# tczhangzhi/pytorch-distributed

Hardware: AMD Instinct MI355X
Metric: ImageNet images/sec (ResNet-50 train step, whole job) (higher is better)
Workload: dtype bf16; 1 GPU; model=resnet50, global_batch=3072, image_size=224, parallelism=dp1, style=ddp, hip_ext=True, hipgraph=False

## Files before the change

amdtrain/models/resnet.py:

```python

from __future__ import annotations

from typing import Callable, Dict, List, Optional, Type, Union

import torch
import torch.nn as nn

from ..ops import fused as OF


import os

from ..ops.conv import AmdConv2d, GradCell, ResidualGradTap
from ..ops.linear import AmdLinear


def _residual_fuse_enabled() -> bool:
    return os.environ.get("AMDTRAIN_RESFUSE", "1") == "1"


def conv3x3(in_planes: int, out_planes: int, stride: int = 1,
            groups: int = 1) -> nn.Conv2d:
    return AmdConv2d(in_planes, out_planes, kernel_size=3, stride=stride,
                     padding=1, groups=groups, bias=False)


def conv1x1(in_planes: int, out_planes: int, stride: int = 1) -> nn.Conv2d:
    return AmdConv2d(in_planes, out_planes, kernel_size=1, stride=stride,
                     bias=False)


class FusedBatchNorm2d(nn.BatchNorm2d):

    def forward(self, x: torch.Tensor) -> torch.Tensor:
        return OF.batch_norm(x, self, relu=False)

    def forward_relu(self, x: torch.Tensor) -> torch.Tensor:
        return OF.batch_norm(x, self, relu=True)


def _shortcut_tail(out: torch.Tensor, bn: FusedBatchNorm2d,
                   downsample: nn.Module, x: torch.Tensor) -> torch.Tensor:
    if (bn.training and isinstance(downsample, nn.Sequential)
            and len(downsample) == 2
            and isinstance(downsample[0], AmdConv2d)
            and isinstance(downsample[1], FusedBatchNorm2d)):
        return OF.bn_add_relu_downsample(out, bn, downsample[0](x),
                                         downsample[1])
    return OF.bn_add_relu(out, bn, downsample(x))


class BasicBlock(nn.Module):
    expansion = 1

    def __init__(self, inplanes: int, planes: int, stride: int = 1,
                 downsample: Optional[nn.Module] = None):
        super().__init__()
        self.conv1 = conv3x3(inplanes, planes, stride)
        self.bn1 = FusedBatchNorm2d(planes)
        self.relu = nn.ReLU(inplace=True)
        self.conv2 = conv3x3(planes, planes)
        self.bn2 = FusedBatchNorm2d(planes)
        self.downsample = downsample
        self.stride = stride

    def forward(self, x: torch.Tensor) -> torch.Tensor:
        identity = x
        cell = None
        if (self.training and x.is_cuda and torch.is_grad_enabled()
                and _residual_fuse_enabled()):
            cell = getattr(x, "_amdtrain_next_cell", None)
        out = self.bn1.forward_relu(self.conv1(x))
        out = self.conv2(out)
        if cell is not None:
            cell.armed = True
            identity = ResidualGradTap.apply(x, cell)
        if self.downsample is not None:
            return _shortcut_tail(out, self.bn2, self.downsample, identity)
        return OF.bn_add_relu(out, self.bn2, identity)


class Bottleneck(nn.Module):
    expansion = 4

    def __init__(self, inplanes: int, planes: int, stride: int = 1,
                 downsample: Optional[nn.Module] = None, groups: int = 1,
                 base_width: int = 64):
        super().__init__()
        width = int(planes * (base_width / 64.0)) * groups
        self.conv1 = conv1x1(inplanes, width)
        self.bn1 = FusedBatchNorm2d(width)
        self.conv2 = conv3x3(width, width, stride, groups)
        self.bn2 = FusedBatchNorm2d(width)
        self.conv3 = conv1x1(width, planes * self.expansion)
        self.bn3 = FusedBatchNorm2d(planes * self.expansion)
        self.relu = nn.ReLU(inplace=True)
        self.downsample = downsample
        self.stride = stride

    def forward(self, x: torch.Tensor) -> torch.Tensor:
        identity = x
        cell = None
        if (self.training and x.is_cuda and torch.is_grad_enabled()
                and _residual_fuse_enabled()):
            cell = getattr(x, "_amdtrain_next_cell", None)
        out = self.bn1.forward_relu(self.conv1(x))
        out = self.bn2.forward_relu(self.conv2(out))
        out = self.conv3(out)
        if cell is not None:
            cell.armed = True
            identity = ResidualGradTap.apply(x, cell)
        if self.downsample is not None:
            return _shortcut_tail(out, self.bn3, self.downsample, identity)
        return OF.bn_add_relu(out, self.bn3, identity)


class ResNet(nn.Module):
    def __init__(self, block: Type[Union[BasicBlock, Bottleneck]],
                 layers: List[int], num_classes: int = 1000,
                 zero_init_residual: bool = False, groups: int = 1,
                 width_per_group: int = 64):
        super().__init__()
        self.groups = groups
        self.base_width = width_per_group
        self.inplanes = 64
        self.conv1 = AmdConv2d(3, 64, kernel_size=7, stride=2, padding=3,
                               bias=False)
        self.bn1 = FusedBatchNorm2d(64)
        self.relu = nn.ReLU(inplace=True)
        self.maxpool = nn.MaxPool2d(kernel_size=3, stride=2, padding=1)
        self.layer1 = self._make_layer(block, 64, layers[0])
        self.layer2 = self._make_layer(block, 128, layers[1], stride=2)
        self.layer3 = self._make_layer(block, 256, layers[2], stride=2)
        self.layer4 = self._make_layer(block, 512, layers[3], stride=2)
        self.avgpool = nn.AdaptiveAvgPool2d((1, 1))
        self.fc = AmdLinear(512 * block.expansion, num_classes)

        for m in self.modules():
            if isinstance(m, nn.Conv2d):
                nn.init.kaiming_normal_(m.weight, mode="fan_out",
                                        nonlinearity="relu")
            elif isinstance(m, nn.BatchNorm2d):
                nn.init.constant_(m.weight, 1)
                nn.init.constant_(m.bias, 0)
        if zero_init_residual:
            for m in self.modules():
                if isinstance(m, Bottleneck):
                    nn.init.constant_(m.bn3.weight, 0)
                elif isinstance(m, BasicBlock):
                    nn.init.constant_(m.bn2.weight, 0)

    def _make_layer(self, block, planes: int, blocks: int,
                    stride: int = 1) -> nn.Sequential:
        downsample = None
        if stride != 1 or self.inplanes != planes * block.expansion:
            downsample = nn.Sequential(
                conv1x1(self.inplanes, planes * block.expansion, stride),
                FusedBatchNorm2d(planes * block.expansion),
            )
        kw = {}
        if block is Bottleneck:
            kw = dict(groups=self.groups, base_width=self.base_width)
        layers = [block(self.inplanes, planes, stride, downsample, **kw)]
        self.inplanes = planes * block.expansion
        for _ in range(1, blocks):
            layers.append(block(self.inplanes, planes, **kw))
        return nn.Sequential(*layers)

    def forward(self, x: torch.Tensor) -> torch.Tensor:
        x = OF.bn_relu_max_pool(self.conv1(x), self.bn1)
        x = self.layer1(x)
        x = self.layer2(x)
        x = self.layer3(x)
        x = self.layer4(x)
        x = OF.global_avg_pool(x)
        x = torch.flatten(x, 1)
        return self.fc(x)


def resnet18(num_classes: int = 1000, **kw) -> ResNet:
    return ResNet(BasicBlock, [2, 2, 2, 2], num_classes=num_classes, **kw)


def resnet34(num_classes: int = 1000, **kw) -> ResNet:
    return ResNet(BasicBlock, [3, 4, 6, 3], num_classes=num_classes, **kw)


def resnet50(num_classes: int = 1000, **kw) -> ResNet:
    return ResNet(Bottleneck, [3, 4, 6, 3], num_classes=num_classes, **kw)


def resnet101(num_classes: int = 1000, **kw) -> ResNet:
    return ResNet(Bottleneck, [3, 4, 23, 3], num_classes=num_classes, **kw)


def resnet152(num_classes: int = 1000, **kw) -> ResNet:
    return ResNet(Bottleneck, [3, 8, 36, 3], num_classes=num_classes, **kw)


def resnext50_32x4d(num_classes: int = 1000, **kw) -> ResNet:
    return ResNet(Bottleneck, [3, 4, 6, 3], num_classes=num_classes,
                  groups=32, width_per_group=4, **kw)


def wide_resnet50_2(num_classes: int = 1000, **kw) -> ResNet:
    return ResNet(Bottleneck, [3, 4, 6, 3], num_classes=num_classes,
                  width_per_group=128, **kw)


_REGISTRY: Dict[str, Callable[..., nn.Module]] = {
    "resnet18": resnet18,
    "resnet34": resnet34,
    "resnet50": resnet50,
    "resnet101": resnet101,
    "resnet152": resnet152,
    "resnext50_32x4d": resnext50_32x4d,
    "wide_resnet50_2": wide_resnet50_2,
}


def model_names() -> List[str]:
    return sorted(_REGISTRY)


def build_model(arch: str, num_classes: int = 1000, **kw) -> nn.Module:
    if arch not in _REGISTRY:
        raise ValueError(f"unknown arch '{arch}'; choices: {model_names()}")
    return _REGISTRY[arch](num_classes=num_classes, **kw)
```

amdtrain/ops/conv.py:

```python

from __future__ import annotations

import os

import torch
import torch.nn as nn

from ._ext import ext_available, require_ext


def _rows(x: torch.Tensor) -> torch.Tensor:
    n, c, h, w = x.shape
    return x.permute(0, 2, 3, 1).reshape(n * h * w, c)


def _fuse_stats_enabled() -> bool:
    return os.environ.get("AMDTRAIN_FUSE_BNSTATS", "1") == "1"


def _wgrad2_enabled() -> bool:
    return os.environ.get("AMDTRAIN_WGRAD2", "1") == "1"


class GradCell:
    __slots__ = ("armed", "g")

    def __init__(self):
        self.armed = False
        self.g = None


class ResidualGradTap(torch.autograd.Function):

    @staticmethod
    def forward(ctx, z: torch.Tensor, cell: "GradCell"):
        ctx.cell = cell
        return z.view_as(z)

    @staticmethod
    def backward(ctx, grad: torch.Tensor):
        if ctx.cell.armed:
            ctx.cell.g = grad
            return None, None
        return grad, None


class _Conv1x1(torch.autograd.Function):

    @staticmethod
    @torch.amp.custom_fwd(device_type="cuda", cast_inputs=torch.bfloat16)
    def forward(ctx, x: torch.Tensor, weight: torch.Tensor, stride: int):
        e = require_ext()
        n, cin, h, w = x.shape
        cout = weight.shape[0]
        xc = x.contiguous(memory_format=torch.channels_last)
        x2d = _rows(xc)
        w2d = weight.reshape(cout, cin)
        stats = None
        if stride > 1:
            y2d = e.gemm_bt_strided(x2d, w2d, n, h, w, stride)
            ho = (h + stride - 1) // stride
            wo = (w + stride - 1) // stride
        elif _fuse_stats_enabled():
            y2d, stats = e.gemm_bt_stats(x2d, w2d)
            ho, wo = h, w
        else:
            y2d = e.gemm_bt(x2d, w2d, False)
            ho, wo = h, w
        ctx.save_for_backward(x2d, w2d)
        ctx.meta = (n, cin, h, w, stride, ho, wo, cout)
        y = y2d.view(n, ho, wo, cout).permute(0, 3, 1, 2)
        if stats is None:
            stats = torch.empty(0, device=x.device)
        ctx.mark_non_differentiable(stats)
        return y, stats

    @staticmethod
    @torch.amp.custom_bwd(device_type="cuda")
    def backward(ctx, grad_y: torch.Tensor, _grad_stats=None):
        e = require_ext()
        x2d, w2d = ctx.saved_tensors
        n, cin, h, w, stride, ho, wo, cout = ctx.meta
        gy = grad_y.contiguous(memory_format=torch.channels_last)
        gy2d = _rows(gy).to(torch.bfloat16)
        wT = e.transpose_2d(w2d)
        dx2d = e.gemm_bt(gy2d, wT, False)
        if stride > 1:
            dx = e.scatter_rows_x2(dx2d, n, h, w, ho, wo)
            dw = e.tn2_wgrad(gy2d, x2d, 1, n, h, w, stride, 1) \
                if _wgrad2_enabled() \
                else e.gemm_tn_strided(gy2d, x2d, n, h, w, stride)
        else:
            dx = dx2d.view(n, ho, wo, cin).permute(0, 3, 1, 2)
            dw = e.tn2_wgrad(gy2d, x2d) if _wgrad2_enabled() \
                else e.gemm_tn(gy2d, x2d, 0)
        return dx, dw.reshape(cout, cin, 1, 1), None


def conv1x1_mfma(x: torch.Tensor, weight: torch.Tensor,
                 stride: int = 1) -> torch.Tensor:
    y, stats = _Conv1x1.apply(x, weight, stride)
    if stats.numel():
        y._amdtrain_bn_stats = stats
    return y


class _Conv3x3(torch.autograd.Function):

    @staticmethod
    @torch.amp.custom_fwd(device_type="cuda", cast_inputs=torch.bfloat16)
    def forward(ctx, x: torch.Tensor, weight: torch.Tensor, stride: int):
        e = require_ext()
        n, cin, h, w = x.shape
        cout = weight.shape[0]
        xc = x.contiguous(memory_format=torch.channels_last)
        x2d = _rows(xc)
        w2d = weight.contiguous(memory_format=torch.channels_last) \
            .permute(0, 2, 3, 1).reshape(cout, 9 * cin)
        if _fuse_stats_enabled():
            y2d, stats = e.conv3x3_fwd_stats(x2d, n, h, w, stride, w2d)
        else:
            y2d = e.conv3x3_fwd(x2d, n, h, w, stride, w2d)
            stats = torch.empty(0, device=x.device)
        ctx.save_for_backward(x2d, w2d)
        ctx.meta = (n, cin, h, w, stride, cout)
        ho = (h + 2 - 3) // stride + 1
        wo = (w + 2 - 3) // stride + 1
        y = y2d.view(n, ho, wo, cout).permute(0, 3, 1, 2)
        ctx.mark_non_differentiable(stats)
        return y, stats

    @staticmethod
    @torch.amp.custom_bwd(device_type="cuda")
    def backward(ctx, grad_y: torch.Tensor, _grad_stats=None):
        e = require_ext()
        x2d, w2d = ctx.saved_tensors
        n, cin, h, w, stride, cout = ctx.meta
        gy = grad_y.contiguous(memory_format=torch.channels_last)
        gy2d = _rows(gy).to(torch.bfloat16)
        dx2d = e.conv3x3_dgrad(gy2d, n, h, w, stride, w2d)
        dx = dx2d.view(n, h, w, cin).permute(0, 3, 1, 2)
        dw2d = e.tn2_wgrad(gy2d, x2d, 9, n, h, w, stride, 2) \
            if _wgrad2_enabled() \
            else e.conv3x3_wgrad(gy2d, x2d, n, h, w, stride)
        dw = dw2d.view(cout, 3, 3, cin).permute(0, 3, 1, 2) \
            .contiguous(memory_format=torch.channels_last)
        return dx, dw, None


def conv3x3_mfma(x: torch.Tensor, weight: torch.Tensor,
                 stride: int = 1) -> torch.Tensor:
    y, stats = _Conv3x3.apply(x, weight, stride)
    if stats.numel():
        y._amdtrain_bn_stats = stats
    return y


class _ConvGrouped3x3(torch.autograd.Function):

    @staticmethod
    @torch.amp.custom_fwd(device_type="cuda", cast_inputs=torch.bfloat16)
    def forward(ctx, x: torch.Tensor, weight: torch.Tensor, stride: int,
                groups: int):
        e = require_ext()
        n, cin, h, w = x.shape
        cout = weight.shape[0]
        sg = cin // groups
        xc = x.contiguous(memory_format=torch.channels_last)
        x2d = _rows(xc)
        sout = cout // groups
        wg = weight.contiguous(memory_format=torch.channels_last) \
            .permute(0, 2, 3, 1).reshape(groups, sout, 3, 3, sg)
        dense = torch.zeros(groups, sout, 3, 3, groups, sg,
                            dtype=wg.dtype, device=wg.device)
        gi = torch.arange(groups, device=wg.device)
        dense[gi, :, :, :, gi, :] = wg
        w2d = dense.reshape(cout, 3, 3, cin).reshape(cout, 9 * cin)
        banded = (cin == cout and cin % 128 == 0)
        if _fuse_stats_enabled():
            y2d, stats = e.conv3x3_fwd_stats(x2d, n, h, w, stride, w2d,
                                             banded)
        else:
            y2d = e.conv3x3_fwd(x2d, n, h, w, stride, w2d)
            stats = torch.empty(0, device=x.device)
        ctx.save_for_backward(x2d, w2d)
        ctx.meta = (n, cin, h, w, stride, cout, groups, banded)
        ho = (h + 2 - 3) // stride + 1
        wo = (w + 2 - 3) // stride + 1
        y = y2d.view(n, ho, wo, cout).permute(0, 3, 1, 2)
        ctx.mark_non_differentiable(stats)
        return y, stats

    @staticmethod
    @torch.amp.custom_bwd(device_type="cuda")
    def backward(ctx, grad_y: torch.Tensor, _grad_stats=None):
        e = require_ext()
        x2d, w2d = ctx.saved_tensors
        n, cin, h, w, stride, cout, groups, banded = ctx.meta
        sg = cin // groups
        sout = cout // groups
        gy = grad_y.contiguous(memory_format=torch.channels_last)
        gy2d = _rows(gy).to(torch.bfloat16)
        dx2d = e.conv3x3_dgrad(gy2d, n, h, w, stride, w2d, banded)
        dx = dx2d.view(n, h, w, cin).permute(0, 3, 1, 2)
        if banded and _wgrad2_enabled():
            dwb = e.tn2_wgrad_banded(gy2d, x2d, n, h, w, stride) \
                .view(cout // 128, 128 // sg, sg, 9, 128 // sg, sg)
            bi = torch.arange(cout // 128, device=dwb.device)[:, None]
            gi = torch.arange(128 // sg, device=dwb.device)[None, :]
            dw = dwb[bi, gi, :, :, gi, :].reshape(cout, 9, sg) \
                .view(cout, 3, 3, sg).permute(0, 3, 1, 2) \
                .contiguous(memory_format=torch.channels_last)
            return dx, dw, None, None
        dw2d = e.tn2_wgrad(gy2d, x2d, 9, n, h, w, stride, 2) \
            if _wgrad2_enabled() \
            else e.conv3x3_wgrad(gy2d, x2d, n, h, w, stride)
        dwd = dw2d.view(groups, sout, 3, 3, groups, sg)
        gi = torch.arange(groups, device=dwd.device)
        dw = dwd[gi, :, :, :, gi, :].permute(0, 1, 4, 2, 3) \
            .reshape(cout, sg, 3, 3) \
            .contiguous(memory_format=torch.channels_last)
        return dx, dw, None, None


def conv3x3_grouped_mfma(x: torch.Tensor, weight: torch.Tensor,
                         stride: int, groups: int) -> torch.Tensor:
    y, stats = _ConvGrouped3x3.apply(x, weight, stride, groups)
    if stats.numel():
        y._amdtrain_bn_stats = stats
    return y


class _ConvGeneric(torch.autograd.Function):

    @staticmethod
    @torch.amp.custom_fwd(device_type="cuda", cast_inputs=torch.bfloat16)
    def forward(ctx, x: torch.Tensor, weight: torch.Tensor, stride: int,
                pad: int):
        e = require_ext()
        n, cin, h, w = x.shape
        cout, _, kh, kw = weight.shape
        xc = x.contiguous(memory_format=torch.channels_last)
        x2d = _rows(xc)
        w4 = weight.contiguous(memory_format=torch.channels_last) \
            .permute(0, 2, 3, 1)
        if cin < 8:
            x2d = torch.nn.functional.pad(x2d, (0, 8 - cin))
            w4 = torch.nn.functional.pad(w4, (0, 8 - cin))
            cin_k = 8
        else:
            cin_k = cin
        k = kh * kw * cin_k
        kpad = (k + 31) // 32 * 32
        w2 = w4.reshape(cout, k)
        if kpad != k:
            w2 = torch.nn.functional.pad(w2, (0, kpad - k))
        y2d = e.conv_generic_fwd(x2d, n, h, w, kh, kw, stride, pad, w2)
        ctx.save_for_backward(x2d, weight)
        ctx.meta = (n, cin, h, w, kh, kw, stride, pad, cout, k, cin_k)
        ho = (h + 2 * pad - kh) // stride + 1
        wo = (w + 2 * pad - kw) // stride + 1
        return y2d.view(n, ho, wo, cout).permute(0, 3, 1, 2)

    @staticmethod
    @torch.amp.custom_bwd(device_type="cuda")
    def backward(ctx, grad_y: torch.Tensor):
        e = require_ext()
        x2d, weight = ctx.saved_tensors
        n, cin, h, w, kh, kw, stride, pad, cout, k, cin_k = ctx.meta
        gy2d = _rows(grad_y.contiguous(memory_format=torch.channels_last)) \
            .to(torch.bfloat16)
        dx = None
        if ctx.needs_input_grad[0]:
            k2 = kh * kw * cout
            k2p = (k2 + 31) // 32 * 32
            w2p = weight.to(torch.bfloat16).permute(1, 2, 3, 0) \
                .reshape(cin, k2)
            if k2p != k2:
                w2p = torch.nn.functional.pad(w2p, (0, k2p - k2))
            dx2d = e.conv_generic_dgrad(gy2d, w2p.contiguous(), n, h, w,
                                        kh, kw, stride, pad)
            dx = dx2d.view(n, h, w, cin).permute(0, 3, 1, 2)
        if _wgrad2_enabled() and cout % 8 == 0:
            dwp = e.tn2_wgrad(gy2d, x2d, kh * kw, n, h, w, stride, 2,
                              kh, kw, pad)
            dw = dwp.view(cout, kh * kw, cin_k)[:, :, :cin] \
                .view(cout, kh, kw, cin).permute(0, 3, 1, 2) \
                .contiguous(memory_format=torch.channels_last)
        else:
            dw2 = e.conv_generic_wgrad(gy2d, x2d, n, h, w, kh, kw, stride,
                                       pad)
            dw = dw2[:, :k].view(cout, kh * kw, cin_k)[:, :, :cin] \
                .reshape(cout, kh, kw, cin).permute(0, 3, 1, 2) \
                .contiguous(memory_format=torch.channels_last)
        return dx, dw, None, None


def conv_stem_mfma(x: torch.Tensor, weight: torch.Tensor, stride: int,
                   pad: int) -> torch.Tensor:
    return _ConvGeneric.apply(x, weight, stride, pad)


def _conv1x1_env_default() -> str:
    return os.environ.get("AMDTRAIN_CONV1X1", "custom")


class AmdConv2d(nn.Conv2d):

    def forward(self, x: torch.Tensor) -> torch.Tensor:
        bf16_ok = (x.dtype == torch.bfloat16
                   or torch.is_autocast_enabled("cuda"))
        if (x.is_cuda and bf16_ok and ext_available()
                and self.bias is None and self.dilation == (1, 1)
                and self.groups > 1):
            if (self.kernel_size == (3, 3) and self.padding == (1, 1)
                    and self.stride[0] in (1, 2)
                    and self.in_channels % 32 == 0
                    and self.out_channels % 16 == 0
                    and self.in_channels % self.groups == 0
                    and os.environ.get("AMDTRAIN_CONV3X3G", "custom")
                    == "custom"):
                return conv3x3_grouped_mfma(x, self.weight, self.stride[0],
                                            self.groups)
            return super().forward(x)
        if (x.is_cuda and bf16_ok and ext_available()
                and self.bias is None and self.groups == 1
                and self.dilation == (1, 1)):
            ch_ok = (self.in_channels % 32 == 0
                     and self.out_channels % 16 == 0)
            if (ch_ok and self.kernel_size == (1, 1)
                    and self.padding == (0, 0)
                    and _conv1x1_env_default() == "custom"):
                return conv1x1_mfma(x, self.weight, self.stride[0])
            if (ch_ok and self.kernel_size == (3, 3)
                    and self.padding == (1, 1)
                    and self.stride[0] in (1, 2)
                    and os.environ.get("AMDTRAIN_CONV3X3", "custom")
                    == "custom"):
                return conv3x3_mfma(x, self.weight, self.stride[0])
            if (self.out_channels % 16 == 0
                    and self.stride[0] == self.stride[1]
                    and self.padding[0] == self.padding[1]
                    and os.environ.get("AMDTRAIN_CONVSTEM", "custom")
                    == "custom"):
                return conv_stem_mfma(x, self.weight, self.stride[0],
                                      self.padding[0])
        return super().forward(x)
```

amdtrain/ops/csrc/batchnorm.hip:

```cpp
#include "common.h"

namespace {

template <typename T>
struct BNDualSide {
  const T* x = nullptr;
  const float* mean = nullptr;
  const float* invstd = nullptr;
  float* out = nullptr;
};

template <typename T, int VEC, bool BWD, int MASK, bool WG, bool GO2,
          bool DUAL = false>
__global__ void __launch_bounds__(AMD_TPB)
bn_reduce_kernel(const T* __restrict__ x, const T* __restrict__ go,
                 const T* __restrict__ goB, const T* __restrict__ y,
                 const float* __restrict__ mean,
                 const float* __restrict__ invstd,
                 const float* __restrict__ scale,
                 const float* __restrict__ shift, T* __restrict__ ghat_out,
                 float* __restrict__ out, long R, int C,
                 BNDualSide<T> ds = {}) {
  static_assert(!DUAL || (BWD && WG), "DUAL rides the ghat-writing bwd pass");
  const int t = threadIdx.x;
  const int gpr = C / VEC;
  const long rows_per_block = (R + gridDim.x - 1) / gridDim.x;
  const long r0 = blockIdx.x * rows_per_block;
  const long r1 = min(r0 + rows_per_block, R);

  if (gpr <= AMD_TPB) {
    const int gc = t % gpr;
    const int phase = t / gpr;
    const int rstep = AMD_TPB / gpr;
    const int c0 = gc * VEC;
    float sa[VEC], sb[VEC];
#pragma unroll
    for (int k = 0; k < VEC; ++k) sa[k] = sb[k] = 0.f;
    float mk[VEC], ik[VEC], sck[VEC], shk[VEC];
    float sda[VEC], sdb[VEC], mdk[VEC], idk[VEC];
    if (BWD) {
#pragma unroll
      for (int k = 0; k < VEC; ++k) {
        mk[k] = mean[c0 + k];
        ik[k] = invstd[c0 + k];
        if (MASK == 2) {
          sck[k] = scale[c0 + k];
          shk[k] = shift[c0 + k];
        }
        if (DUAL) {
          sda[k] = sdb[k] = 0.f;
          mdk[k] = ds.mean[c0 + k];
          idk[k] = ds.invstd[c0 + k];
        }
      }
    }
    for (long r = r0 + phase; r < r1; r += rstep) {
      const long base = r * C + c0;
      Pack<T, VEC> xv = *(const Pack<T, VEC>*)(x + base);
      Pack<T, VEC> gv, gv2, yv, gh, dv;
      unsigned int mbits = 0;
      if (BWD) {
        gv = *(const Pack<T, VEC>*)(go + base);
        if (DUAL) dv = *(const Pack<T, VEC>*)(ds.x + base);
        if (GO2) gv2 = *(const Pack<T, VEC>*)(goB + base);
        if (MASK == 1) yv = *(const Pack<T, VEC>*)(y + base);
        if (MASK == 3)
          mbits = ((const unsigned char*)y)[base / VEC];
      }
#pragma unroll
      for (int k = 0; k < VEC; ++k) {
        float xe = to_f32(xv.v[k]);
        if (BWD) {
          float ge = to_f32(gv.v[k]);
          if (GO2) ge += to_f32(gv2.v[k]);
          if (MASK == 1 && to_f32(yv.v[k]) <= 0.f) ge = 0.f;
          if (MASK == 2 && sck[k] * xe + shk[k] <= 0.f) ge = 0.f;
          if (MASK == 3 && !(mbits & (1u << k))) ge = 0.f;
          sa[k] += ge;
          sb[k] += ge * (xe - mk[k]) * ik[k];
          if (WG) gh.v[k] = from_f32<T>(ge);
          if (DUAL) {
            const float gr = to_f32(gh.v[k]);
            sda[k] += gr;
            sdb[k] += gr * (to_f32(dv.v[k]) - mdk[k]) * idk[k];
          }
        } else {
          sa[k] += xe;
          sb[k] += xe * xe;
        }
      }
      if (BWD && WG) *(Pack<T, VEC>*)(ghat_out + base) = gh;
    }
    __shared__ float lds[AMD_TPB * VEC];
    auto fold = [&](float(&s)[VEC]) {
#pragma unroll
      for (int k = 0; k < VEC; ++k) lds[t * VEC + k] = s[k];
      __syncthreads();
      if (phase == 0) {
        for (int ph = 1; ph < rstep; ++ph)
#pragma unroll
          for (int k = 0; k < VEC; ++k)
            s[k] += lds[(ph * gpr + gc) * VEC + k];
      }
      __syncthreads();
    };
    fold(sa);
    fold(sb);
    if (DUAL) {
      fold(sda);
      fold(sdb);
    }
    if (phase == 0) {
      float* part = out + (long)blockIdx.x * 2 * C;
#pragma unroll
      for (int k = 0; k < VEC; ++k) {
        part[c0 + k] = sa[k];
        part[C + c0 + k] = sb[k];
      }
      if (DUAL) {
        float* partd = ds.out + (long)blockIdx.x * 2 * C;
#pragma unroll
        for (int k = 0; k < VEC; ++k) {
          partd[c0 + k] = sda[k];
          partd[C + c0 + k] = sdb[k];
        }
      }
    }
  } else {
    const int cpt = gpr / AMD_TPB;
    float sa[2][VEC], sb[2][VEC];
    float mk[2][VEC], ik[2][VEC], sck[2][VEC], shk[2][VEC];
#pragma unroll
    for (int j = 0; j < 2; ++j)
#pragma unroll
      for (int k = 0; k < VEC; ++k) {
        sa[j][k] = sb[j][k] = 0.f;
        if (BWD && j < cpt) {
          mk[j][k] = mean[(t + j * AMD_TPB) * VEC + k];
          ik[j][k] = invstd[(t + j * AMD_TPB) * VEC + k];
          if (MASK == 2) {
            sck[j][k] = scale[(t + j * AMD_TPB) * VEC + k];
            shk[j][k] = shift[(t + j * AMD_TPB) * VEC + k];
          }
        }
      }
    for (long r = r0; r < r1; ++r) {
      for (int j = 0; j < cpt; ++j) {
        const int c0 = (t + j * AMD_TPB) * VEC;
        const long base = r * C + c0;
        Pack<T, VEC> xv = *(const Pack<T, VEC>*)(x + base);
        Pack<T, VEC> gv, gv2, yv, gh;
        unsigned int mbits = 0;
        if (BWD) {
          gv = *(const Pack<T, VEC>*)(go + base);
          if (GO2) gv2 = *(const Pack<T, VEC>*)(goB + base);
          if (MASK == 1) yv = *(const Pack<T, VEC>*)(y + base);
          if (MASK == 3)
            mbits = ((const unsigned char*)y)[base / VEC];
        }
#pragma unroll
        for (int k = 0; k < VEC; ++k) {
          float xe = to_f32(xv.v[k]);
          if (BWD) {
            float ge = to_f32(gv.v[k]);
            if (GO2) ge += to_f32(gv2.v[k]);
            if (MASK == 1 && to_f32(yv.v[k]) <= 0.f) ge = 0.f;
            if (MASK == 2 && sck[j][k] * xe + shk[j][k] <= 0.f) ge = 0.f;
            if (MASK == 3 && !(mbits & (1u << k))) ge = 0.f;
            sa[j][k] += ge;
            sb[j][k] += ge * (xe - mk[j][k]) * ik[j][k];
            if (WG) gh.v[k] = from_f32<T>(ge);
          } else {
            sa[j][k] += xe;
            sb[j][k] += xe * xe;
          }
        }
        if (BWD && WG) *(Pack<T, VEC>*)(ghat_out + base) = gh;
      }
    }
    float* part = out + (long)blockIdx.x * 2 * C;
    for (int j = 0; j < cpt; ++j) {
      const int c0 = (t + j * AMD_TPB) * VEC;
#pragma unroll
      for (int k = 0; k < VEC; ++k) {
        part[c0 + k] = sa[j][k];
        part[C + c0 + k] = sb[j][k];
      }
    }
  }
}

constexpr int BN_COLLAPSE = 32;

static inline int bn_collapse_slots(int nparts) {
  return nparts >= 2048 ? 4 * BN_COLLAPSE : BN_COLLAPSE;
}

__global__ void bn_collapse_partials_kernel(const float* __restrict__ in,
                                            float* __restrict__ out,
                                            int nparts, int twoC, int slots) {
  const int slot = blockIdx.x % slots;
  const int cblk = blockIdx.x / slots;
  const int c = cblk * AMD_TPB + threadIdx.x;
  if (c >= twoC) return;
  float acc = 0.f;
  for (int p = slot; p < nparts; p += slots)
    acc += in[(long)p * twoC + c];
  out[(long)slot * twoC + c] = acc;
}

__global__ void bn_finalize_train_kernel(
    const float* __restrict__ partials, int nparts,
    const float* __restrict__ w,
    const float* __restrict__ b, float* __restrict__ rm,
    float* __restrict__ rv, float* __restrict__ mean,
    float* __restrict__ invstd, float* __restrict__ scale,
    float* __restrict__ shift, long R, int C, float momentum, float eps) {
  const int c = blockIdx.x * 64 + (threadIdx.x & 63);
  const int sl = threadIdx.x >> 6;
  float s1 = 0.f, s2 = 0.f;
  if (c < C)
    for (int p = sl; p < nparts; p += 4) {
      s1 += partials[(long)p * 2 * C + c];
      s2 += partials[(long)p * 2 * C + C + c];
    }
  __shared__ float red[2][4][64];
  red[0][sl][threadIdx.x & 63] = s1;
  red[1][sl][threadIdx.x & 63] = s2;
  __syncthreads();
  if (sl != 0 || c >= C) return;
  s1 += red[0][1][threadIdx.x] + red[0][2][threadIdx.x] +
        red[0][3][threadIdx.x];
  s2 += red[1][1][threadIdx.x] + red[1][2][threadIdx.x] +
        red[1][3][threadIdx.x];
  float m = s1 / R;
  float var = fmaxf(s2 / R - m * m, 0.f);
  float is = rsqrtf(var + eps);
  mean[c] = m;
  invstd[c] = is;
  float unbiased = R > 1 ? var * (float)R / (float)(R - 1) : var;
  rm[c] = (1.f - momentum) * rm[c] + momentum * m;
  rv[c] = (1.f - momentum) * rv[c] + momentum * unbiased;
  float sc = w[c] * is;
  scale[c] = sc;
  shift[c] = b[c] - m * sc;
}

__global__ void bn_finalize_eval_kernel(
    const float* __restrict__ w, const float* __restrict__ b,
    const float* __restrict__ rm, const float* __restrict__ rv,
    float* __restrict__ scale, float* __restrict__ shift, int C, float eps) {
  int c = blockIdx.x * blockDim.x + threadIdx.x;
  if (c >= C) return;
  float is = rsqrtf(rv[c] + eps);
  float sc = w[c] * is;
  scale[c] = sc;
  shift[c] = b[c] - rm[c] * sc;
}

template <typename T, int VEC, bool RELU, bool HAS_ADD, bool POW2,
          bool DUAL = false>
__global__ void __launch_bounds__(AMD_TPB)
bn_apply_kernel(const T* __restrict__ x, const T* __restrict__ z,
                T* __restrict__ y, unsigned char* __restrict__ mask,
                const float* __restrict__ scale,
                const float* __restrict__ shift, long total_vec, int C,
                const float* __restrict__ scale_d = nullptr,
                const float* __restrict__ shift_d = nullptr) {
  static_assert(!DUAL || (HAS_ADD && POW2), "DUAL normalizes the addend");
  extern __shared__ float sm[];
  const int gpr = C / VEC;
  const long stride = (long)gridDim.x * blockDim.x;
  float rs[VEC], rb[VEC], rsd[VEC], rbd[VEC];
  if (DUAL) {
    const int cf =
        (int)(((long)blockIdx.x * blockDim.x + threadIdx.x) & (gpr - 1)) * VEC;
#pragma unroll
    for (int k = 0; k < VEC; ++k) {
      rs[k] = scale[cf + k];
      rb[k] = shift[cf + k];
      rsd[k] = scale_d[cf + k];
      rbd[k] = shift_d[cf + k];
    }
  } else {
    for (int c = threadIdx.x; c < C; c += blockDim.x) {
      sm[c] = scale[c];
      sm[C + c] = shift[c];
    }
    __syncthreads();
  }
  for (long i = (long)blockIdx.x * blockDim.x + threadIdx.x; i < total_vec;
       i += 2 * stride) {
    const bool has2 = i + stride < total_vec;
    const long i2 = has2 ? i + stride : i;
    Pack<T, VEC> xv = *(const Pack<T, VEC>*)(x + i * VEC);
    Pack<T, VEC> xv2 = *(const Pack<T, VEC>*)(x + i2 * VEC);
    Pack<T, VEC> zv, zv2;
    if (HAS_ADD) {
      zv = *(const Pack<T, VEC>*)(z + i * VEC);
      zv2 = *(const Pack<T, VEC>*)(z + i2 * VEC);
    }
    const int c0 = (int)(POW2 ? (i & (gpr - 1)) : (i % gpr)) * VEC;
    const int c02 = (int)(POW2 ? (i2 & (gpr - 1)) : (i2 % gpr)) * VEC;
    Pack<T, VEC> yv, yv2;
    unsigned int mb = 0, mb2 = 0;
#pragma unroll
    for (int k = 0; k < VEC; ++k) {
      float v = DUAL ? rs[k] * to_f32(xv.v[k]) + rb[k]
                     : sm[c0 + k] * to_f32(xv.v[k]) + sm[C + c0 + k];
      if (HAS_ADD) {
        float ze = to_f32(zv.v[k]);
        if (DUAL) ze = to_f32(from_f32<T>(rsd[k] * ze + rbd[k]));
        v += ze;
      }
      if (RELU) {
        if (mask != nullptr && v > 0.f) mb |= 1u << k;
        v = fmaxf(v, 0.f);
      }
      yv.v[k] = from_f32<T>(v);
      float v2 = DUAL ? rs[k] * to_f32(xv2.v[k]) + rb[k]
                      : sm[c02 + k] * to_f32(xv2.v[k]) + sm[C + c02 + k];
      if (HAS_ADD) {
        float ze2 = to_f32(zv2.v[k]);
        if (DUAL) ze2 = to_f32(from_f32<T>(rsd[k] * ze2 + rbd[k]));
        v2 += ze2;
      }
      if (RELU) {
        if (mask != nullptr && v2 > 0.f) mb2 |= 1u << k;
        v2 = fmaxf(v2, 0.f);
      }
      yv2.v[k] = from_f32<T>(v2);
    }
    *(Pack<T, VEC>*)(y + i * VEC) = yv;
    if (has2) *(Pack<T, VEC>*)(y + i2 * VEC) = yv2;
    if (RELU && mask != nullptr) {
      mask[i] = (unsigned char)mb;
      if (has2) mask[i2] = (unsigned char)mb2;
    }
  }
}

__global__ void bn_bwd_finalize_kernel(
    const float* __restrict__ partials, int nparts,
    const float* __restrict__ w, const float* __restrict__ mean,
    const float* __restrict__ invstd, float* __restrict__ gw,
    float* __restrict__ gb, float* __restrict__ A, float* __restrict__ Bc,
    float* __restrict__ Dc, long R, int C) {
  const int c = blockIdx.x * 64 + (threadIdx.x & 63);
  const int sl = threadIdx.x >> 6;
  float sg = 0.f, sgx = 0.f;
  if (c < C)
    for (int p = sl; p < nparts; p += 4) {
      sg += partials[(long)p * 2 * C + c];
      sgx += partials[(long)p * 2 * C + C + c];
    }
  __shared__ float red[2][4][64];
  red[0][sl][threadIdx.x & 63] = sg;
  red[1][sl][threadIdx.x & 63] = sgx;
  __syncthreads();
  if (sl != 0 || c >= C) return;
  sg += red[0][1][threadIdx.x] + red[0][2][threadIdx.x] +
        red[0][3][threadIdx.x];
  sgx += red[1][1][threadIdx.x] + red[1][2][threadIdx.x] +
         red[1][3][threadIdx.x];
  gb[c] = sg;
  gw[c] = sgx;
  float a = w[c] * invstd[c];
  float bcoef = -a * invstd[c] * sgx / R;
  A[c] = a;
  Bc[c] = bcoef;
  Dc[c] = -a * sg / R - bcoef * mean[c];
}

template <typename T>
struct BNDualBwdSide {
  const T* x = nullptr;
  T* gx = nullptr;
  const float* A = nullptr;
  const float* Bc = nullptr;
  const float* Dc = nullptr;
};

template <typename T, int VEC, int MASK, bool WRITE_GHAT, bool POW2,
          bool DUAL = false>
__global__ void __launch_bounds__(AMD_TPB)
bn_bwd_apply_kernel(const T* __restrict__ x, const T* __restrict__ go,
                    T* __restrict__ gx,
                    T* __restrict__ ghat_out, const float* __restrict__ A,
                    const float* __restrict__ Bc, const float* __restrict__ Dc,
                    const float* __restrict__ scale,
                    const float* __restrict__ shift, long total_vec, int C,
                    BNDualBwdSide<T> ds = {}) {
  static_assert(!DUAL || (MASK == 0 && POW2 && !WRITE_GHAT),
                "DUAL consumes the materialized ghat");
  const int gpr = C / VEC;
  const long stride = (long)gridDim.x * blockDim.x;
  if (DUAL) {
    const long i0 = (long)blockIdx.x * blockDim.x + threadIdx.x;
    const int c0 = (int)(i0 & (gpr - 1)) * VEC;
    float a3[VEC], b3[VEC], d3[VEC], ad[VEC], bd[VEC], dd[VEC];
#pragma unroll
    for (int k = 0; k < VEC; ++k) {
      a3[k] = A[c0 + k];
      b3[k] = Bc[c0 + k];
      d3[k] = Dc[c0 + k];
      ad[k] = ds.A[c0 + k];
      bd[k] = ds.Bc[c0 + k];
      dd[k] = ds.Dc[c0 + k];
    }
    for (long i = i0; i < total_vec; i += 2 * stride) {
      const bool has2 = i + stride < total_vec;
      const long i2 = has2 ? i + stride : i;
      Pack<T, VEC> xv = *(const Pack<T, VEC>*)(x + i * VEC);
      Pack<T, VEC> dv = *(const Pack<T, VEC>*)(ds.x + i * VEC);
      Pack<T, VEC> gv = *(const Pack<T, VEC>*)(go + i * VEC);
      Pack<T, VEC> xv2 = *(const Pack<T, VEC>*)(x + i2 * VEC);
      Pack<T, VEC> dv2 = *(const Pack<T, VEC>*)(ds.x + i2 * VEC);
      Pack<T, VEC> gv2 = *(const Pack<T, VEC>*)(go + i2 * VEC);
      Pack<T, VEC> out, dout, out2, dout2;
#pragma unroll
      for (int k = 0; k < VEC; ++k) {
        float ge = to_f32(gv.v[k]);
        float v = a3[k] * ge + b3[k] * to_f32(xv.v[k]) + d3[k];
        out.v[k] = from_f32<T>(v);
        float w = ad[k] * ge + bd[k] * to_f32(dv.v[k]) + dd[k];
        dout.v[k] = from_f32<T>(w);
        float ge2 = to_f32(gv2.v[k]);
        float v2 = a3[k] * ge2 + b3[k] * to_f32(xv2.v[k]) + d3[k];
        out2.v[k] = from_f32<T>(v2);
        float w2 = ad[k] * ge2 + bd[k] * to_f32(dv2.v[k]) + dd[k];
        dout2.v[k] = from_f32<T>(w2);
      }
      *(Pack<T, VEC>*)(gx + i * VEC) = out;
      *(Pack<T, VEC>*)(ds.gx + i * VEC) = dout;
      if (has2) {
        *(Pack<T, VEC>*)(gx + i2 * VEC) = out2;
        *(Pack<T, VEC>*)(ds.gx + i2 * VEC) = dout2;
      }
    }
    return;
  }
  extern __shared__ float sm[];
  for (int c = threadIdx.x; c < C; c += blockDim.x) {
    sm[c] = A[c];
    sm[C + c] = Bc[c];
    sm[2 * C + c] = Dc[c];
    if (MASK == 2) {
      sm[3 * C + c] = scale[c];
      sm[4 * C + c] = shift[c];
    }
  }
  __syncthreads();
  for (long i = (long)blockIdx.x * blockDim.x + threadIdx.x; i < total_vec;
       i += 2 * stride) {
    const bool has2 = i + stride < total_vec;
    const long i2 = has2 ? i + stride : i;
    Pack<T, VEC> xv = *(const Pack<T, VEC>*)(x + i * VEC);
    Pack<T, VEC> gv = *(const Pack<T, VEC>*)(go + i * VEC);
    Pack<T, VEC> xv2 = *(const Pack<T, VEC>*)(x + i2 * VEC);
    Pack<T, VEC> gv2 = *(const Pack<T, VEC>*)(go + i2 * VEC);
    const int c0 = (int)(POW2 ? (i & (gpr - 1)) : (i % gpr)) * VEC;
    const int c02 = (int)(POW2 ? (i2 & (gpr - 1)) : (i2 % gpr)) * VEC;
    Pack<T, VEC> out, gh, out2, gh2;
#pragma unroll
    for (int k = 0; k < VEC; ++k) {
      float xe = to_f32(xv.v[k]);
      float ge = to_f32(gv.v[k]);
      if (MASK == 2 && sm[3 * C + c0 + k] * xe + sm[4 * C + c0 + k] <= 0.f)
        ge = 0.f;
      float v = sm[c0 + k] * ge + sm[C + c0 + k] * xe + sm[2 * C + c0 + k];
      out.v[k] = from_f32<T>(v);
      if (WRITE_GHAT) gh.v[k] = from_f32<T>(ge);
      float xe2 = to_f32(xv2.v[k]);
      float ge2 = to_f32(gv2.v[k]);
      if (MASK == 2 && sm[3 * C + c02 + k] * xe2 + sm[4 * C + c02 + k] <= 0.f)
        ge2 = 0.f;
      float v2 = sm[c02 + k] * ge2 + sm[C + c02 + k] * xe2 +
                 sm[2 * C + c02 + k];
      out2.v[k] = from_f32<T>(v2);
      if (WRITE_GHAT) gh2.v[k] = from_f32<T>(ge2);
    }
    *(Pack<T, VEC>*)(gx + i * VEC) = out;
    if (WRITE_GHAT) *(Pack<T, VEC>*)(ghat_out + i * VEC) = gh;
    if (has2) {
      *(Pack<T, VEC>*)(gx + i2 * VEC) = out2;
      if (WRITE_GHAT) *(Pack<T, VEC>*)(ghat_out + i2 * VEC) = gh2;
    }
  }
}


static void check_nhwc(const at::Tensor& x) {
  TORCH_CHECK(x.is_cuda() && x.dim() == 4, "expected 4D CUDA tensor");
  TORCH_CHECK(x.is_contiguous(at::MemoryFormat::ChannelsLast),
              "expected channels_last (NHWC) tensor");
}

template <typename F>
static void dispatch_vec(const at::Tensor& x, F fn) {
  int C = (int)x.size(1);
  AT_DISPATCH_FLOATING_TYPES_AND2(
      at::ScalarType::BFloat16, at::ScalarType::Half, x.scalar_type(), "bn",
      [&] {
        using devT = typename DevT<scalar_t>::type;
        constexpr int VEC = 16 / sizeof(devT);
        TORCH_CHECK(C % VEC == 0, "C must be a multiple of ", VEC);
        TORCH_CHECK((C & (C - 1)) == 0,
                    "C must be a power of two (apply-kernel fast path): ", C);
        TORCH_CHECK(C / VEC <= 2 * AMD_TPB, "C too large: ", C);
        fn((devT*)nullptr, std::integral_constant<int, VEC>{});
      });
}

static int bn_reduce_grid(long R, int C) {
  long rows_per_block = std::max<long>(1, R / 1536);
  return (int)std::min<long>((R + rows_per_block - 1) / rows_per_block, 1536);
}

static at::Tensor bn_collapse(const at::Tensor& parts, long C,
                              hipStream_t stream) {
  const int nparts = (int)parts.size(0);
  const int slots = bn_collapse_slots(nparts);
  auto sums2 = at::empty({slots, 2 * C}, parts.options());
  int cgrid = slots * (int)((2 * C + AMD_TPB - 1) / AMD_TPB);
  bn_collapse_partials_kernel<<<cgrid, AMD_TPB, 0, stream>>>(
      parts.data_ptr<float>(), sums2.data_ptr<float>(), nparts, (int)(2 * C),
      slots);
  CHECK_CUDA_OK();
  return sums2;
}

struct BNTrainStats {
  at::Tensor mean, invstd, scale, shift;
};

static BNTrainStats bn_train_stats(const at::Tensor& x,
                                   const std::optional<at::Tensor>& parts,
                                   const at::Tensor& weight,
                                   const at::Tensor& bias,
                                   at::Tensor& running_mean,
                                   at::Tensor& running_var, double momentum,
                                   double eps) {
  const long C = x.size(1);
  const long R = x.numel() / C;
  auto opts = x.options().dtype(at::kFloat);
  auto stream = at::cuda::getCurrentCUDAStream();
  at::Tensor sums;
  if (parts) {
    TORCH_CHECK(parts->size(1) == 2 * C, "parts must be [nparts][2C]");
    sums = *parts;
  } else {
    const int rgrid = bn_reduce_grid(R, C);
    sums = at::empty({rgrid, 2 * C}, opts);
    dispatch_vec(x, [&](auto* tp, auto vec) {
      using devT = std::remove_pointer_t<decltype(tp)>;
      constexpr int VEC = decltype(vec)::value;
      bn_reduce_kernel<devT, VEC, false, 0, false, false>
          <<<rgrid, AMD_TPB, 0, stream>>>((const devT*)x.const_data_ptr(),
                                          nullptr, nullptr, nullptr, nullptr,
                                          nullptr, nullptr, nullptr, nullptr,
                                          sums.data_ptr<float>(), R, (int)C);
      CHECK_CUDA_OK();
    });
  }
  auto sums2 = bn_collapse(sums, C, stream);
  BNTrainStats s{at::empty({C}, opts), at::empty({C}, opts),
                 at::empty({C}, opts), at::empty({C}, opts)};
  int fgrid = (int)((C + 63) / 64);
  bn_finalize_train_kernel<<<fgrid, AMD_TPB, 0, stream>>>(
      sums2.data_ptr<float>(), (int)sums2.size(0), weight.data_ptr<float>(),
      bias.data_ptr<float>(), running_mean.data_ptr<float>(),
      running_var.data_ptr<float>(), s.mean.data_ptr<float>(),
      s.invstd.data_ptr<float>(), s.scale.data_ptr<float>(),
      s.shift.data_ptr<float>(), R, (int)C, (float)momentum, (float)eps);
  CHECK_CUDA_OK();
  return s;
}

struct BNBwdCoeffs {
  at::Tensor gw, gb, A, Bc, Dc;
};

static BNBwdCoeffs bn_bwd_coeffs(const at::Tensor& sums,
                                 const at::Tensor& weight,
                                 const at::Tensor& mean,
                                 const at::Tensor& invstd, long R, long C) {
  auto stream = at::cuda::getCurrentCUDAStream();
  auto opts = sums.options();
  auto sums2 = bn_collapse(sums, C, stream);
  BNBwdCoeffs k{at::empty({C}, opts), at::empty({C}, opts),
                at::empty({C}, opts), at::empty({C}, opts),
                at::empty({C}, opts)};
  int fgrid = (int)((C + 63) / 64);
  bn_bwd_finalize_kernel<<<fgrid, AMD_TPB, 0, stream>>>(
      sums2.data_ptr<float>(), (int)sums2.size(0), weight.data_ptr<float>(),
      mean.data_ptr<float>(), invstd.data_ptr<float>(),
      k.gw.data_ptr<float>(), k.gb.data_ptr<float>(), k.A.data_ptr<float>(),
      k.Bc.data_ptr<float>(), k.Dc.data_ptr<float>(), R, (int)C);
  CHECK_CUDA_OK();
  return k;
}

static void check_dual(const at::Tensor& x3, const at::Tensor& x_d) {
  check_nhwc(x3);
  check_nhwc(x_d);
  TORCH_CHECK(x3.sizes() == x_d.sizes() &&
                  x3.scalar_type() == x_d.scalar_type(),
              "dual BN tail: x3 and x_d must match in shape and dtype");
  TORCH_CHECK(x3.size(1) * (long)x3.element_size() / 16 <= AMD_TPB,
              "dual BN tail: C too wide for the register path: ", x3.size(1));
}

}

std::vector<at::Tensor> batch_norm_train_stats(
    at::Tensor x, std::optional<at::Tensor> parts, at::Tensor weight,
    at::Tensor bias, at::Tensor running_mean, at::Tensor running_var,
    double momentum, double eps) {
  check_nhwc(x);
  auto s = bn_train_stats(x, parts, weight, bias, running_mean, running_var,
                          momentum, eps);
  return {s.mean, s.invstd, s.scale, s.shift};
}

std::vector<at::Tensor> batch_norm_fwd_train(
    at::Tensor x, at::Tensor weight, at::Tensor bias, at::Tensor running_mean,
    at::Tensor running_var, double momentum, double eps, bool relu,
    std::optional<at::Tensor> addend) {
  check_nhwc(x);
  const long N = x.size(0), C = x.size(1), H = x.size(2), W = x.size(3);
  const long R = N * H * W;
  auto y = at::empty_like(x);
  at::Tensor mask;
  if (relu && addend)
    mask = at::empty({R * C / 4}, x.options().dtype(at::kByte));
  auto stream = at::cuda::getCurrentCUDAStream();
  auto st = bn_train_stats(x, std::nullopt, weight, bias, running_mean,
                           running_var, momentum, eps);
  auto &mean = st.mean, &invstd = st.invstd, &scale = st.scale,
       &shift = st.shift;

  dispatch_vec(x, [&](auto* tp, auto vec) {
    using devT = std::remove_pointer_t<decltype(tp)>;
    constexpr int VEC = decltype(vec)::value;
    long total_vec = R * C / VEC;
    int agrid = amd_grid(total_vec);
    size_t smem = 2 * C * sizeof(float);
    const devT* zp =
        addend ? (const devT*)addend->const_data_ptr() : nullptr;
#define APPLY(RELU_, ADD_)                                                  \
  bn_apply_kernel<devT, VEC, RELU_, ADD_, true>                             \
      <<<agrid, AMD_TPB, smem, stream>>>(                                   \
          (const devT*)x.const_data_ptr(), zp, (devT*)y.data_ptr(),         \
          mask.defined() ? mask.data_ptr<unsigned char>() : nullptr,        \
          scale.data_ptr<float>(), shift.data_ptr<float>(),     \
          total_vec, (int)C)
    if (relu && addend) APPLY(true, true);
    else if (relu) APPLY(true, false);
    else if (addend) APPLY(false, true);
    else APPLY(false, false);
#undef APPLY
    CHECK_CUDA_OK();
  });
  if (!mask.defined()) mask = at::empty({0}, x.options().dtype(at::kByte));
  return {y, mean, invstd, scale, shift, mask};
}

std::vector<at::Tensor> batch_norm_fwd_train_from_parts(
    at::Tensor x, at::Tensor parts, at::Tensor weight, at::Tensor bias,
    at::Tensor running_mean, at::Tensor running_var, double momentum,
    double eps, bool relu, std::optional<at::Tensor> addend) {
  check_nhwc(x);
  const long C = x.size(1);
  const long R = x.numel() / C;
  auto y = at::empty_like(x);
  at::Tensor mask;
  if (relu && addend)
    mask = at::empty({R * C / 4}, x.options().dtype(at::kByte));
  auto stream = at::cuda::getCurrentCUDAStream();
  auto st = bn_train_stats(x, parts, weight, bias, running_mean, running_var,
                           momentum, eps);
  auto &mean = st.mean, &invstd = st.invstd, &scale = st.scale,
       &shift = st.shift;
  dispatch_vec(x, [&](auto* tp, auto vec) {
    using devT = std::remove_pointer_t<decltype(tp)>;
    constexpr int VEC = decltype(vec)::value;
    long total_vec = R * C / VEC;
    int agrid = amd_grid(total_vec);
    size_t smem = 2 * C * sizeof(float);
    const devT* zp =
        addend ? (const devT*)addend->const_data_ptr() : nullptr;
#define APPLY2(RELU_, ADD_)                                                 \
  bn_apply_kernel<devT, VEC, RELU_, ADD_, true>                             \
      <<<agrid, AMD_TPB, smem, stream>>>(                                   \
          (const devT*)x.const_data_ptr(), zp, (devT*)y.data_ptr(),         \
          mask.defined() ? mask.data_ptr<unsigned char>() : nullptr,        \
          scale.data_ptr<float>(), shift.data_ptr<float>(),                 \
          total_vec, (int)C)
    if (relu && addend) APPLY2(true, true);
    else if (relu) APPLY2(true, false);
    else if (addend) APPLY2(false, true);
    else APPLY2(false, false);
#undef APPLY2
    CHECK_CUDA_OK();
  });
  if (!mask.defined()) mask = at::empty({0}, x.options().dtype(at::kByte));
  return {y, mean, invstd, scale, shift, mask};
}

std::vector<at::Tensor> batch_norm_dual_fwd_train(
    at::Tensor x3, at::Tensor x_d, std::optional<at::Tensor> parts3,
    std::optional<at::Tensor> parts_d, at::Tensor weight3, at::Tensor bias3,
    at::Tensor running_mean3, at::Tensor running_var3, double momentum3,
    double eps3, at::Tensor weight_d, at::Tensor bias_d,
    at::Tensor running_mean_d, at::Tensor running_var_d, double momentum_d,
    double eps_d) {
  check_dual(x3, x_d);
  const long C = x3.size(1);
  const long R = x3.numel() / C;
  auto sd = bn_train_stats(x_d, parts_d, weight_d, bias_d, running_mean_d,
                           running_var_d, momentum_d, eps_d);
  auto s3 = bn_train_stats(x3, parts3, weight3, bias3, running_mean3,
                           running_var3, momentum3, eps3);
  auto y = at::empty_like(x3);
  auto mask = at::empty({R * C / 4}, x3.options().dtype(at::kByte));
  auto stream = at::cuda::getCurrentCUDAStream();
  dispatch_vec(x3, [&](auto* tp, auto vec) {
    using devT = std::remove_pointer_t<decltype(tp)>;
    constexpr int VEC = decltype(vec)::value;
    long total_vec = R * C / VEC;
    int agrid = amd_grid(total_vec);
    bn_apply_kernel<devT, VEC, true, true, true, true>
        <<<agrid, AMD_TPB, 0, stream>>>(
            (const devT*)x3.const_data_ptr(),
            (const devT*)x_d.const_data_ptr(), (devT*)y.data_ptr(),
            mask.data_ptr<unsigned char>(), s3.scale.data_ptr<float>(),
            s3.shift.data_ptr<float>(), total_vec, (int)C,
            sd.scale.data_ptr<float>(), sd.shift.data_ptr<float>());
    CHECK_CUDA_OK();
  });
  return {y, s3.mean, s3.invstd, sd.mean, sd.invstd, mask};
}

std::vector<at::Tensor> batch_norm_dual_bwd(
    at::Tensor x3, at::Tensor x_d, at::Tensor grad_out,
    std::optional<at::Tensor> grad_out2, at::Tensor relu_mask,
    at::Tensor weight3, at::Tensor mean3, at::Tensor invstd3,
    at::Tensor weight_d, at::Tensor mean_d, at::Tensor invstd_d) {
  check_dual(x3, x_d);
  check_nhwc(grad_out);
  const long C = x3.size(1);
  const long R = x3.numel() / C;
  TORCH_CHECK(relu_mask.numel() == R * C / 4, "relu_mask size mismatch");
  auto opts = x3.options().dtype(at::kFloat);
  const int rgrid = bn_reduce_grid(R, C);
  auto sums3 = at::empty({rgrid, 2 * C}, opts);
  auto sums_d = at::empty({rgrid, 2 * C}, opts);
  auto ghat = at::empty_like(grad_out);
  auto gx3 = at::empty_like(x3);
  auto gx_d = at::empty_like(x_d);
  BNBwdCoeffs k3, kd;
  auto stream = at::cuda::getCurrentCUDAStream();
  dispatch_vec(x3, [&](auto* tp, auto vec) {
    using devT = std::remove_pointer_t<decltype(tp)>;
    constexpr int VEC = decltype(vec)::value;
    const devT* go2p = grad_out2
        ? (const devT*)grad_out2->const_data_ptr() : nullptr;
    BNDualSide<devT> rs{(const devT*)x_d.const_data_ptr(),
                        mean_d.data_ptr<float>(), invstd_d.data_ptr<float>(),
                        sums_d.data_ptr<float>()};
#define REDUCE_DUAL(GO2_)                                                   \
  bn_reduce_kernel<devT, VEC, true, 3, true, GO2_, true>                    \
      <<<rgrid, AMD_TPB, 0, stream>>>(                                      \
          (const devT*)x3.const_data_ptr(),                                 \
          (const devT*)grad_out.const_data_ptr(), go2p,                     \
          (const devT*)relu_mask.const_data_ptr(), mean3.data_ptr<float>(), \
          invstd3.data_ptr<float>(), nullptr, nullptr,                      \
          (devT*)ghat.data_ptr(), sums3.data_ptr<float>(), R, (int)C, rs)
    if (go2p) REDUCE_DUAL(true);
    else REDUCE_DUAL(false);
#undef REDUCE_DUAL
    CHECK_CUDA_OK();
    k3 = bn_bwd_coeffs(sums3, weight3, mean3, invstd3, R, C);
    kd = bn_bwd_coeffs(sums_d, weight_d, mean_d, invstd_d, R, C);
    long total_vec = R * C / VEC;
    int agrid = amd_grid(total_vec);
    BNDualBwdSide<devT> as{(const devT*)x_d.const_data_ptr(),
                           (devT*)gx_d.data_ptr(), kd.A.data_ptr<float>(),
                           kd.Bc.data_ptr<float>(), kd.Dc.data_ptr<float>()};
    bn_bwd_apply_kernel<devT, VEC, 0, false, true, true>
        <<<agrid, AMD_TPB, 0, stream>>>(
            (const devT*)x3.const_data_ptr(),
            (const devT*)ghat.const_data_ptr(), (devT*)gx3.data_ptr(),
            nullptr, k3.A.data_ptr<float>(), k3.Bc.data_ptr<float>(),
            k3.Dc.data_ptr<float>(), nullptr, nullptr, total_vec, (int)C, as);
    CHECK_CUDA_OK();
  });
  return {gx3, k3.gw, k3.gb, gx_d, kd.gw, kd.gb};
}

at::Tensor batch_norm_fwd_eval(at::Tensor x, at::Tensor weight,
                               at::Tensor bias, at::Tensor running_mean,
                               at::Tensor running_var, double eps, bool relu,
                               std::optional<at::Tensor> addend) {
  check_nhwc(x);
  const long C = x.size(1);
  const long R = x.numel() / C;
  auto opts = x.options().dtype(at::kFloat);
  auto scale = at::empty({C}, opts);
  auto shift = at::empty({C}, opts);
  auto y = at::empty_like(x);
  at::Tensor mask;
  auto stream = at::cuda::getCurrentCUDAStream();
  int fgrid = (int)((C + AMD_TPB - 1) / AMD_TPB);
  bn_finalize_eval_kernel<<<fgrid, AMD_TPB, 0, stream>>>(
      weight.data_ptr<float>(), bias.data_ptr<float>(),
      running_mean.data_ptr<float>(), running_var.data_ptr<float>(),
      scale.data_ptr<float>(), shift.data_ptr<float>(), (int)C, (float)eps);
  CHECK_CUDA_OK();
  dispatch_vec(x, [&](auto* tp, auto vec) {
    using devT = std::remove_pointer_t<decltype(tp)>;
    constexpr int VEC = decltype(vec)::value;
    long total_vec = R * C / VEC;
    int agrid = amd_grid(total_vec);
    size_t smem = 2 * C * sizeof(float);
    const devT* zp =
        addend ? (const devT*)addend->const_data_ptr() : nullptr;
#define APPLY(RELU_, ADD_)                                                  \
  bn_apply_kernel<devT, VEC, RELU_, ADD_, true>                             \
      <<<agrid, AMD_TPB, smem, stream>>>(                                   \
          (const devT*)x.const_data_ptr(), zp, (devT*)y.data_ptr(),         \
          mask.defined() ? mask.data_ptr<unsigned char>() : nullptr,        \
          scale.data_ptr<float>(), shift.data_ptr<float>(),     \
          total_vec, (int)C)
    if (relu && addend) APPLY(true, true);
    else if (relu) APPLY(true, false);
    else if (addend) APPLY(false, true);
    else APPLY(false, false);
#undef APPLY
    CHECK_CUDA_OK();
  });
  return y;
}

std::vector<at::Tensor> batch_norm_bwd(at::Tensor x, at::Tensor grad_out,
                                       std::optional<at::Tensor> y,
                                       at::Tensor weight,
                                       at::Tensor mean, at::Tensor invstd,
                                       bool relu, bool need_ghat,
                                       std::optional<at::Tensor> scale,
                                       std::optional<at::Tensor> shift,
                                       std::optional<at::Tensor> grad_out2,
                                       std::optional<at::Tensor> relu_mask) {
  check_nhwc(x);
  check_nhwc(grad_out);
  const long C = x.size(1);
  const long R = x.numel() / C;
  auto opts = x.options().dtype(at::kFloat);
  const int rgrid = bn_reduce_grid(R, C);
  auto sums = at::empty({rgrid, 2 * C}, opts);
  BNBwdCoeffs k;
  auto gx = at::empty_like(x);
  const bool affine_mask = relu && !need_ghat && scale && shift;
  const bool mask_y = relu && (!affine_mask || grad_out2.has_value());
  at::Tensor ghat;
  if (mask_y || grad_out2) ghat = at::empty_like(grad_out);
  auto stream = at::cuda::getCurrentCUDAStream();

  dispatch_vec(x, [&](auto* tp, auto vec) {
    using devT = std::remove_pointer_t<decltype(tp)>;
    constexpr int VEC = decltype(vec)::value;
    const float* scp = affine_mask ? scale->data_ptr<float>() : nullptr;
    const float* shp = affine_mask ? shift->data_ptr<float>() : nullptr;
    const devT* go2p = grad_out2
        ? (const devT*)grad_out2->const_data_ptr() : nullptr;
#define REDUCE(MASK_, WG_, GO2_)                                            \
  bn_reduce_kernel<devT, VEC, true, MASK_, WG_, GO2_>                       \
      <<<rgrid, AMD_TPB, 0, stream>>>(                                      \
          (const devT*)x.const_data_ptr(),                                  \
          (const devT*)grad_out.const_data_ptr(), go2p,                     \
          yp, mean.data_ptr<float>(),                                       \
          invstd.data_ptr<float>(), scp, shp,                               \
          WG_ ? (devT*)ghat.data_ptr() : nullptr,                           \
          sums.data_ptr<float>(), R, (int)C)
#define REDUCE3(GO2_)                                                       \
  bn_reduce_kernel<devT, VEC, true, 3, true, GO2_>                          \
      <<<rgrid, AMD_TPB, 0, stream>>>(                                      \
          (const devT*)x.const_data_ptr(),                                  \
          (const devT*)grad_out.const_data_ptr(), go2p,                     \
          (const devT*)mkp, mean.data_ptr<float>(),                         \
          invstd.data_ptr<float>(), scp, shp,                               \
          (devT*)ghat.data_ptr(),                                           \
          sums.data_ptr<float>(), R, (int)C)
    const unsigned char* mkp = (relu_mask && relu_mask->numel())
        ? relu_mask->data_ptr<unsigned char>() : nullptr;
    TORCH_CHECK(y.has_value() || !mask_y || mkp,
                "batch_norm_bwd: y is required to mask a relu+addend BN "
                "that saved no relu_mask");
    const devT* yp = y ? (const devT*)y->const_data_ptr() : nullptr;
    if (mask_y && mkp && go2p) REDUCE3(true);
    else if (mask_y && mkp) REDUCE3(false);
    else if (mask_y && go2p) REDUCE(1, true, true);
    else if (mask_y) REDUCE(1, true, false);
    else if (affine_mask) REDUCE(2, false, false);
    else if (go2p) REDUCE(0, true, true);
    else REDUCE(0, false, false);
#undef REDUCE
#undef REDUCE3
    CHECK_CUDA_OK();
    k = bn_bwd_coeffs(sums, weight, mean, invstd, R, C);
    long total_vec = R * C / VEC;
    int agrid = amd_grid(total_vec);
    size_t smem = (affine_mask ? 5 : 3) * C * sizeof(float);
    const devT* go_in = ghat.defined()
                            ? (const devT*)ghat.const_data_ptr()
                            : (const devT*)grad_out.const_data_ptr();
#define BAPPLY(MASK_)                                                       \
  bn_bwd_apply_kernel<devT, VEC, MASK_, false, true>                        \
      <<<agrid, AMD_TPB, smem, stream>>>(                                   \
          (const devT*)x.const_data_ptr(), go_in, (devT*)gx.data_ptr(),     \
          nullptr, k.A.data_ptr<float>(), k.Bc.data_ptr<float>(),           \
          k.Dc.data_ptr<float>(), scp, shp, total_vec, (int)C)
    if (affine_mask) BAPPLY(2);
    else BAPPLY(0);
#undef BAPPLY
    CHECK_CUDA_OK();
  });
  if (!ghat.defined()) ghat = grad_out;
  return {gx, k.gw, k.gb, ghat};
}
```

amdtrain/ops/csrc/ext.cpp:

```cpp
#include <torch/extension.h>

#include <optional>
#include <vector>

void multi_tensor_sgd(std::vector<at::Tensor> params,
                      std::vector<at::Tensor> grads,
                      std::vector<at::Tensor> momenta, double lr,
                      double momentum, double weight_decay, bool nesterov,
                      bool first, bool zero_grad);

std::vector<at::Tensor> cross_entropy_fwd(at::Tensor logits, at::Tensor target);
at::Tensor cross_entropy_bwd(at::Tensor logits, at::Tensor target,
                             at::Tensor lse, at::Tensor upstream);

at::Tensor normalize_u8(at::Tensor x, std::vector<double> mean,
                        std::vector<double> std_, long dtype_code);
at::Tensor topk_ranks(at::Tensor logits, at::Tensor target);
at::Tensor scatter_rows_x2(at::Tensor src2d, long Nn, long H, long W,
                           long Hs, long Ws);
void multi_tensor_scale_check(std::vector<at::Tensor> tensors, double scale,
                              at::Tensor found_inf);
void multi_tensor_cast(std::vector<at::Tensor> src,
                       std::vector<at::Tensor> dst);

std::vector<at::Tensor> batch_norm_fwd_train(
    at::Tensor x, at::Tensor weight, at::Tensor bias, at::Tensor running_mean,
    at::Tensor running_var, double momentum, double eps, bool relu,
    std::optional<at::Tensor> addend);
std::vector<at::Tensor> batch_norm_fwd_train_from_parts(
    at::Tensor x, at::Tensor parts, at::Tensor weight, at::Tensor bias,
    at::Tensor running_mean, at::Tensor running_var, double momentum,
    double eps, bool relu, std::optional<at::Tensor> addend);
at::Tensor batch_norm_fwd_eval(at::Tensor x, at::Tensor weight,
                               at::Tensor bias, at::Tensor running_mean,
                               at::Tensor running_var, double eps, bool relu,
                               std::optional<at::Tensor> addend);
std::vector<at::Tensor> batch_norm_train_stats(
    at::Tensor x, std::optional<at::Tensor> parts, at::Tensor weight,
    at::Tensor bias, at::Tensor running_mean, at::Tensor running_var,
    double momentum, double eps);
std::vector<at::Tensor> batch_norm_dual_fwd_train(
    at::Tensor x3, at::Tensor x_d, std::optional<at::Tensor> parts3,
    std::optional<at::Tensor> parts_d, at::Tensor weight3, at::Tensor bias3,
    at::Tensor running_mean3, at::Tensor running_var3, double momentum3,
    double eps3, at::Tensor weight_d, at::Tensor bias_d,
    at::Tensor running_mean_d, at::Tensor running_var_d, double momentum_d,
    double eps_d);
std::vector<at::Tensor> batch_norm_dual_bwd(
    at::Tensor x3, at::Tensor x_d, at::Tensor grad_out,
    std::optional<at::Tensor> grad_out2, at::Tensor relu_mask,
    at::Tensor weight3, at::Tensor mean3, at::Tensor invstd3,
    at::Tensor weight_d, at::Tensor mean_d, at::Tensor invstd_d);
std::vector<at::Tensor> batch_norm_bwd(at::Tensor x, at::Tensor grad_out,
                                       std::optional<at::Tensor> y,
                                       at::Tensor weight,
                                       at::Tensor mean, at::Tensor invstd,
                                       bool relu, bool need_ghat,
                                       std::optional<at::Tensor> scale,
                                       std::optional<at::Tensor> shift,
                                       std::optional<at::Tensor> grad_out2,
                                       std::optional<at::Tensor> relu_mask);

at::Tensor gemm_bt(at::Tensor A, at::Tensor B, bool f32_out,
                   std::optional<at::Tensor> addend,
                   std::optional<at::Tensor> bias);
at::Tensor gemm_tn(at::Tensor dY, at::Tensor X, long msplit);
at::Tensor gemm_bt_strided(at::Tensor A, at::Tensor B, long Nn, long H,
                           long W, long stride);
at::Tensor gemm_tn_strided(at::Tensor dY, at::Tensor X, long Nn, long H,
                           long W, long stride);
at::Tensor transpose_2d(at::Tensor x);

at::Tensor conv3x3_fwd(at::Tensor x2d, long Nn, long H, long W, long stride,
                       at::Tensor w2d);
std::vector<at::Tensor> conv3x3_fwd_stats(at::Tensor x2d, long Nn, long H,
                                          long W, long stride,
                                          at::Tensor w2d, bool banded);
std::vector<at::Tensor> gemm_bt_stats(at::Tensor A, at::Tensor B);

at::Tensor gemm_bt_8p(at::Tensor A, at::Tensor B);
at::Tensor gemm_bt_8p3(at::Tensor A, at::Tensor B);
at::Tensor conv3x3_8p(at::Tensor A2d, long Nn, long H, long W, long stride,
                      at::Tensor w2d, bool dgrad);
at::Tensor conv3x3_dgrad(at::Tensor dy2d, long Nn, long H, long W,
                         long stride, at::Tensor w2d, bool banded);
at::Tensor conv3x3_wgrad(at::Tensor dy2d, at::Tensor x2d, long Nn, long H,
                         long W, long stride);

at::Tensor tn2_wgrad(at::Tensor dY, at::Tensor X, long taps, long Nn, long H,
                     long W, long stride, long gmode, long kh, long kw,
                     long pad);
at::Tensor tn2_wgrad_banded(at::Tensor dY, at::Tensor X, long Nn, long H,
                            long W, long stride);
at::Tensor tr16_probe(at::Tensor in);

at::Tensor conv_generic_fwd(at::Tensor x2d, long Nn, long H, long W, long KH,
                            long KW, long stride, long pad, at::Tensor w2);
at::Tensor conv_generic_wgrad(at::Tensor dy2d, at::Tensor x2d, long Nn,
                              long H, long W, long KH, long KW, long stride,
                              long pad);
at::Tensor conv_generic_dgrad(at::Tensor dy2d, at::Tensor w2p, long Nn,
                              long H, long W, long KH, long KW, long stride,
                              long pad);

std::vector<at::Tensor> max_pool_3x3_s2_fwd(at::Tensor x,
                                            std::optional<at::Tensor> scale,
                                            std::optional<at::Tensor> shift);
at::Tensor max_pool_3x3_s2_bwd(at::Tensor grad_y, at::Tensor idx, long H,
                               long W);
at::Tensor global_avg_pool_fwd(at::Tensor x);
at::Tensor global_avg_pool_bwd(at::Tensor grad_y, long H, long W);

PYBIND11_MODULE(TORCH_EXTENSION_NAME, m) {
  m.doc() = "amdtrain hand-written gfx950 (CDNA4) HIP kernels";
  m.def("multi_tensor_sgd", &multi_tensor_sgd, "fused multi-tensor SGD");
  m.def("cross_entropy_fwd", &cross_entropy_fwd);
  m.def("cross_entropy_bwd", &cross_entropy_bwd);
  m.def("normalize_u8", &normalize_u8);
  m.def("topk_ranks", &topk_ranks);
  m.def("scatter_rows_x2", &scatter_rows_x2);
  m.def("multi_tensor_scale_check", &multi_tensor_scale_check);
  m.def("multi_tensor_cast", &multi_tensor_cast);
  m.def("batch_norm_fwd_train", &batch_norm_fwd_train,
        py::arg("x"), py::arg("weight"), py::arg("bias"),
        py::arg("running_mean"), py::arg("running_var"), py::arg("momentum"),
        py::arg("eps"), py::arg("relu"),
        py::arg("addend") = std::nullopt);
  m.def("batch_norm_fwd_train_from_parts", &batch_norm_fwd_train_from_parts,
        py::arg("x"), py::arg("parts"), py::arg("weight"), py::arg("bias"),
        py::arg("running_mean"), py::arg("running_var"), py::arg("momentum"),
        py::arg("eps"), py::arg("relu"), py::arg("addend") = std::nullopt);
  m.def("batch_norm_fwd_eval", &batch_norm_fwd_eval,
        py::arg("x"), py::arg("weight"), py::arg("bias"),
        py::arg("running_mean"), py::arg("running_var"), py::arg("eps"),
        py::arg("relu"), py::arg("addend") = std::nullopt);
  m.def("batch_norm_train_stats", &batch_norm_train_stats);
  m.def("batch_norm_dual_fwd_train", &batch_norm_dual_fwd_train);
  m.def("batch_norm_dual_bwd", &batch_norm_dual_bwd);
  m.def("batch_norm_bwd", &batch_norm_bwd, py::arg("x"), py::arg("grad_out"),
        py::arg("y"), py::arg("weight"), py::arg("mean"), py::arg("invstd"),
        py::arg("relu"), py::arg("need_ghat"),
        py::arg("scale") = std::nullopt, py::arg("shift") = std::nullopt,
        py::arg("grad_out2") = std::nullopt,
        py::arg("relu_mask") = std::nullopt);
  m.def("gemm_bt", &gemm_bt, py::arg("A"), py::arg("B"),
        py::arg("f32_out") = false, py::arg("addend") = std::nullopt,
        py::arg("bias") = std::nullopt);
  m.def("gemm_tn", &gemm_tn, py::arg("dY"), py::arg("X"),
        py::arg("msplit") = 0);
  m.def("gemm_bt_strided", &gemm_bt_strided);
  m.def("gemm_tn_strided", &gemm_tn_strided);
  m.def("transpose_2d", &transpose_2d);
  m.def("conv3x3_fwd", &conv3x3_fwd);
  m.def("conv3x3_fwd_stats", &conv3x3_fwd_stats, py::arg("x2d"),
        py::arg("Nn"), py::arg("H"), py::arg("W"), py::arg("stride"),
        py::arg("w2d"), py::arg("banded") = false);
  m.def("gemm_bt_stats", &gemm_bt_stats);
  m.def("gemm_bt_8p", &gemm_bt_8p);
  m.def("gemm_bt_8p3", &gemm_bt_8p3);
  m.def("conv3x3_8p", &conv3x3_8p);
  m.def("conv3x3_dgrad", &conv3x3_dgrad, py::arg("dy2d"), py::arg("Nn"),
        py::arg("H"), py::arg("W"), py::arg("stride"), py::arg("w2d"),
        py::arg("banded") = false);
  m.def("conv3x3_wgrad", &conv3x3_wgrad);
  m.def("tn2_wgrad", &tn2_wgrad, py::arg("dY"), py::arg("X"),
        py::arg("taps") = 1, py::arg("Nn") = 0, py::arg("H") = 0,
        py::arg("W") = 0, py::arg("stride") = 1, py::arg("gmode") = 0,
        py::arg("kh") = 3, py::arg("kw") = 3, py::arg("pad") = 1);
  m.def("tn2_wgrad_banded", &tn2_wgrad_banded);
  m.def("tr16_probe", &tr16_probe);
  m.def("conv_generic_fwd", &conv_generic_fwd);
  m.def("conv_generic_wgrad", &conv_generic_wgrad);
  m.def("conv_generic_dgrad", &conv_generic_dgrad);
  m.def("max_pool_3x3_s2_fwd", &max_pool_3x3_s2_fwd, py::arg("x"),
        py::arg("scale") = std::nullopt, py::arg("shift") = std::nullopt);
  m.def("max_pool_3x3_s2_bwd", &max_pool_3x3_s2_bwd);
  m.def("global_avg_pool_fwd", &global_avg_pool_fwd);
  m.def("global_avg_pool_bwd", &global_avg_pool_bwd);
}
```

amdtrain/ops/fused.py:

```python

from __future__ import annotations

import os
from typing import Optional

import torch
import torch.nn.functional as F

from ._ext import require_ext, use_ext_for
from .conv import GradCell

__all__ = ["batch_norm", "bn_add_relu", "bn_add_relu_downsample",
           "bn_relu_max_pool", "max_pool_3x3_s2", "global_avg_pool"]


class _BNFunction(torch.autograd.Function):

    @staticmethod
    def forward(ctx, x, weight, bias, running_mean, running_var,
                momentum, eps, relu, addend, parts, res_cell=None):
        e = require_ext()
        if parts is not None:
            y, mean, invstd, scale, shift, mask = \
                e.batch_norm_fwd_train_from_parts(
                    x, parts, weight, bias, running_mean, running_var,
                    float(momentum), float(eps), bool(relu), addend)
        else:
            y, mean, invstd, scale, shift, mask = e.batch_norm_fwd_train(
                x, weight, bias, running_mean, running_var,
                float(momentum), float(eps), bool(relu), addend)
        ctx.save_for_backward(x, y, weight, mean, invstd, scale, shift,
                              mask)
        ctx.relu = bool(relu)
        ctx.has_addend = addend is not None
        ctx.res_cell = res_cell
        return y

    @staticmethod
    def backward(ctx, grad_out):
        x, y, weight, mean, invstd, scale, shift, mask = ctx.saved_tensors
        e = require_ext()
        go2 = None
        cell = getattr(ctx, "res_cell", None)
        if cell is not None and cell.g is not None:
            go2 = cell.g.contiguous(memory_format=torch.channels_last)
            cell.g = None
        grad_x, grad_w, grad_b, ghat = e.batch_norm_bwd(
            x, grad_out.contiguous(memory_format=torch.channels_last),
            y, weight, mean, invstd, ctx.relu, ctx.has_addend,
            scale, shift, go2, mask)
        grad_addend = ghat if ctx.has_addend else None
        return (grad_x, grad_w, grad_b, None, None, None, None, None,
                grad_addend, None, None)


def _bn_torch(x: torch.Tensor, bn, relu: bool,
              addend: Optional[torch.Tensor]) -> torch.Tensor:
    y = F.batch_norm(
        x, bn.running_mean, bn.running_var, bn.weight, bn.bias,
        bn.training or not bn.track_running_stats,
        bn.momentum if bn.momentum is not None else 0.0, bn.eps)
    if addend is not None:
        y = y + addend
    if relu:
        y = F.relu(y, inplace=True)
    return y


def batch_norm(x: torch.Tensor, bn, relu: bool = False,
               addend: Optional[torch.Tensor] = None) -> torch.Tensor:
    if bn.training and bn.track_running_stats and bn.num_batches_tracked is not None:
        bn.num_batches_tracked.add_(1)
    C = x.size(1)
    if use_ext_for(x) and (C & (C - 1)) == 0:
        parts = getattr(x, "_amdtrain_bn_stats", None) if bn.training else None
        xc = x.contiguous(memory_format=torch.channels_last)
        ac = None if addend is None else addend.contiguous(memory_format=torch.channels_last)
        if bn.training:
            cell = GradCell() if (relu and ac is not None) else None
            out = _BNFunction.apply(xc, bn.weight, bn.bias, bn.running_mean,
                                    bn.running_var, bn.momentum, bn.eps,
                                    relu, ac, parts, cell)
            if cell is not None:
                out._amdtrain_next_cell = cell
            return out
        return require_ext().batch_norm_fwd_eval(
            xc, bn.weight, bn.bias, bn.running_mean, bn.running_var,
            float(bn.eps), bool(relu), ac)
    return _bn_torch(x, bn, relu, addend)


def bn_add_relu(x: torch.Tensor, bn, addend: torch.Tensor) -> torch.Tensor:
    return batch_norm(x, bn, relu=True, addend=addend)


class _BNDualFunction(torch.autograd.Function):

    @staticmethod
    def forward(ctx, x3, x_d, weight3, bias3, running_mean3, running_var3,
                momentum3, eps3, weight_d, bias_d, running_mean_d,
                running_var_d, momentum_d, eps_d, parts3, parts_d, res_cell):
        e = require_ext()
        y, mean3, invstd3, mean_d, invstd_d, mask = \
            e.batch_norm_dual_fwd_train(
                x3, x_d, parts3, parts_d,
                weight3, bias3, running_mean3, running_var3,
                float(momentum3), float(eps3),
                weight_d, bias_d, running_mean_d, running_var_d,
                float(momentum_d), float(eps_d))
        ctx.save_for_backward(x3, x_d, weight3, mean3, invstd3, weight_d,
                              mean_d, invstd_d, mask)
        ctx.res_cell = res_cell
        return y

    @staticmethod
    def backward(ctx, grad_out):
        (x3, x_d, weight3, mean3, invstd3, weight_d, mean_d, invstd_d,
         mask) = ctx.saved_tensors
        e = require_ext()
        go2 = None
        cell = getattr(ctx, "res_cell", None)
        if cell is not None and cell.g is not None:
            go2 = cell.g.contiguous(memory_format=torch.channels_last)
            cell.g = None
        gx3, gw3, gb3, gx_d, gw_d, gb_d = e.batch_norm_dual_bwd(
            x3, x_d, grad_out.contiguous(memory_format=torch.channels_last),
            go2, mask, weight3, mean3, invstd3, weight_d, mean_d, invstd_d)
        return (gx3, gx_d, gw3, gb3, None, None, None, None, gw_d, gb_d,
                None, None, None, None, None, None, None)


def _dsfuse_enabled() -> bool:
    return os.environ.get("AMDTRAIN_DSFUSE", "1") == "1"


def _stemfuse_enabled() -> bool:
    return os.environ.get("AMDTRAIN_STEMFUSE", "1") == "1"


def _vec_ok(x: torch.Tensor, max_groups: int) -> bool:
    C = x.size(1)
    vec = 16 // x.element_size()
    return (C & (C - 1)) == 0 and C % vec == 0 and C // vec <= max_groups


def bn_add_relu_downsample(x3: torch.Tensor, bn3, x_d: torch.Tensor,
                           bn_d) -> torch.Tensor:
    if (bn3.training and bn_d.training and _dsfuse_enabled()
            and use_ext_for(x3) and x3.shape == x_d.shape
            and x3.dtype == x_d.dtype and _vec_ok(x3, 256)):
        for bn in (bn_d, bn3):
            if bn.track_running_stats and bn.num_batches_tracked is not None:
                bn.num_batches_tracked.add_(1)
        parts3 = getattr(x3, "_amdtrain_bn_stats", None)
        parts_d = getattr(x_d, "_amdtrain_bn_stats", None)
        cell = GradCell()
        out = _BNDualFunction.apply(
            x3.contiguous(memory_format=torch.channels_last),
            x_d.contiguous(memory_format=torch.channels_last),
            bn3.weight, bn3.bias, bn3.running_mean, bn3.running_var,
            bn3.momentum, bn3.eps, bn_d.weight, bn_d.bias,
            bn_d.running_mean, bn_d.running_var, bn_d.momentum, bn_d.eps,
            parts3, parts_d, cell)
        out._amdtrain_next_cell = cell
        return out
    return bn_add_relu(x3, bn3, batch_norm(x_d, bn_d))


class _MaxPool3x3S2(torch.autograd.Function):
    @staticmethod
    def forward(ctx, x):
        e = require_ext()
        y, idx = e.max_pool_3x3_s2_fwd(x)
        ctx.save_for_backward(idx)
        ctx.in_shape = x.shape
        return y

    @staticmethod
    def backward(ctx, grad_out):
        (idx,) = ctx.saved_tensors
        e = require_ext()
        n, c, h, w = ctx.in_shape
        gx = e.max_pool_3x3_s2_bwd(
            grad_out.contiguous(memory_format=torch.channels_last), idx,
            int(h), int(w))
        return gx


def max_pool_3x3_s2(x: torch.Tensor) -> torch.Tensor:
    if use_ext_for(x):
        return _MaxPool3x3S2.apply(x.contiguous(memory_format=torch.channels_last))
    return F.max_pool2d(x, kernel_size=3, stride=2, padding=1)


class _BNReLUMaxPool(torch.autograd.Function):

    @staticmethod
    def forward(ctx, x, weight, bias, running_mean, running_var, momentum,
                eps, parts):
        e = require_ext()
        mean, invstd, scale, shift = e.batch_norm_train_stats(
            x, parts, weight, bias, running_mean, running_var,
            float(momentum), float(eps))
        y, idx = e.max_pool_3x3_s2_fwd(x, scale, shift)
        ctx.save_for_backward(x, idx, weight, mean, invstd, scale, shift)
        return y

    @staticmethod
    def backward(ctx, grad_out):
        x, idx, weight, mean, invstd, scale, shift = ctx.saved_tensors
        e = require_ext()
        gp = e.max_pool_3x3_s2_bwd(
            grad_out.contiguous(memory_format=torch.channels_last), idx,
            int(x.size(2)), int(x.size(3)))
        grad_x, grad_w, grad_b, _ = e.batch_norm_bwd(
            x, gp, None, weight, mean, invstd, True, False, scale, shift,
            None, None)
        return grad_x, grad_w, grad_b, None, None, None, None, None


def bn_relu_max_pool(x: torch.Tensor, bn) -> torch.Tensor:
    if (bn.training and _stemfuse_enabled() and use_ext_for(x)
            and _vec_ok(x, 512)):
        if bn.track_running_stats and bn.num_batches_tracked is not None:
            bn.num_batches_tracked.add_(1)
        parts = getattr(x, "_amdtrain_bn_stats", None)
        return _BNReLUMaxPool.apply(
            x.contiguous(memory_format=torch.channels_last), bn.weight,
            bn.bias, bn.running_mean, bn.running_var, bn.momentum, bn.eps,
            parts)
    return max_pool_3x3_s2(batch_norm(x, bn, relu=True))


class _GlobalAvgPool(torch.autograd.Function):
    @staticmethod
    def forward(ctx, x):
        e = require_ext()
        y = e.global_avg_pool_fwd(x)
        ctx.in_shape = x.shape
        return y

    @staticmethod
    def backward(ctx, grad_out):
        e = require_ext()
        n, c, h, w = ctx.in_shape
        return e.global_avg_pool_bwd(grad_out.contiguous(), int(h), int(w))


def global_avg_pool(x: torch.Tensor) -> torch.Tensor:
    if use_ext_for(x):
        return _GlobalAvgPool.apply(x.contiguous(memory_format=torch.channels_last))
    return F.adaptive_avg_pool2d(x, (1, 1))
```

Measured before the change: 10140 images/sec.

## Fuse maxpool backward into stem BN backward and keep stride-2 downsample grads compact

The stem's BN+ReLU+maxpool backward now gathers pool gradients directly inside the BN reduce and apply kernels. The residual gradient from layer1's first block is also folded in through a grad cell, so the separate pool-backward pass and the add disappear. For stride-2 downsample 1x1 convs, the input gradient is left in compact (unscattered) form and read by the preceding BN backward via a strided gather, avoiding the scatter_rows_x2 materialization. BN apply and backward-apply gain a register-resident coefficient path. Together these add index-decoding arithmetic and extra kernel template variants, and they carry correctness risk at odd-position rows and edges.

```diff
diff --git a/amdtrain/models/resnet.py b/amdtrain/models/resnet.py
--- a/amdtrain/models/resnet.py
+++ b/amdtrain/models/resnet.py
@@ -11,7 +11,8 @@
 
 import os
 
-from ..ops.conv import AmdConv2d, GradCell, ResidualGradTap
+from ..ops.conv import (AmdConv2d, GradCell, ResidualGradTap,
+                        tap_residual)
 from ..ops.linear import AmdLinear
 
 
@@ -74,7 +75,7 @@
         out = self.conv2(out)
         if cell is not None:
             cell.armed = True
-            identity = ResidualGradTap.apply(x, cell)
+            identity = tap_residual(x, cell)
         if self.downsample is not None:
             return _shortcut_tail(out, self.bn2, self.downsample, identity)
         return OF.bn_add_relu(out, self.bn2, identity)
@@ -109,7 +110,7 @@
         out = self.conv3(out)
         if cell is not None:
             cell.armed = True
-            identity = ResidualGradTap.apply(x, cell)
+            identity = tap_residual(x, cell)
         if self.downsample is not None:
             return _shortcut_tail(out, self.bn3, self.downsample, identity)
         return OF.bn_add_relu(out, self.bn3, identity)
diff --git a/amdtrain/ops/conv.py b/amdtrain/ops/conv.py
--- a/amdtrain/ops/conv.py
+++ b/amdtrain/ops/conv.py
@@ -23,11 +23,17 @@
 
 
 class GradCell:
-    __slots__ = ("armed", "g")
+    __slots__ = ("armed", "g", "compact_ok", "meta")
 
     def __init__(self):
         self.armed = False
         self.g = None
+        self.compact_ok = False
+        self.meta = None
+
+
+def _dsgrad_compact_enabled() -> bool:
+    return os.environ.get("AMDTRAIN_DSGRAD_COMPACT", "1") == "1"
 
 
 class ResidualGradTap(torch.autograd.Function):
@@ -35,21 +41,32 @@
     @staticmethod
     def forward(ctx, z: torch.Tensor, cell: "GradCell"):
         ctx.cell = cell
+        ctx.set_materialize_grads(False)
         return z.view_as(z)
 
     @staticmethod
-    def backward(ctx, grad: torch.Tensor):
+    def backward(ctx, grad):
+        if grad is None:
+            return None, None
         if ctx.cell.armed:
             ctx.cell.g = grad
+            ctx.cell.meta = None
             return None, None
         return grad, None
 
 
+def tap_residual(x: torch.Tensor, cell: "GradCell") -> torch.Tensor:
+    out = ResidualGradTap.apply(x, cell)
+    out._amdtrain_tap_cell = cell
+    return out
+
+
 class _Conv1x1(torch.autograd.Function):
 
     @staticmethod
     @torch.amp.custom_fwd(device_type="cuda", cast_inputs=torch.bfloat16)
-    def forward(ctx, x: torch.Tensor, weight: torch.Tensor, stride: int):
+    def forward(ctx, x: torch.Tensor, weight: torch.Tensor, stride: int,
+                cell=None):
         e = require_ext()
         n, cin, h, w = x.shape
         cout = weight.shape[0]
@@ -57,6 +74,7 @@
         x2d = _rows(xc)
         w2d = weight.reshape(cout, cin)
         stats = None
+        ctx.cell = cell
         if stride > 1:
             y2d = e.gemm_bt_strided(x2d, w2d, n, h, w, stride)
             ho = (h + stride - 1) // stride
@@ -86,7 +104,14 @@
         wT = e.transpose_2d(w2d)
         dx2d = e.gemm_bt(gy2d, wT, False)
         if stride > 1:
-            dx = e.scatter_rows_x2(dx2d, n, h, w, ho, wo)
+            cell = ctx.cell
+            if (stride == 2 and cell is not None and cell.armed
+                    and cell.compact_ok):
+                cell.g = dx2d
+                cell.meta = (n, h, w, ho, wo)
+                dx = None
+            else:
+                dx = e.scatter_rows_x2(dx2d, n, h, w, ho, wo)
             dw = e.tn2_wgrad(gy2d, x2d, 1, n, h, w, stride, 1) \
                 if _wgrad2_enabled() \
                 else e.gemm_tn_strided(gy2d, x2d, n, h, w, stride)
@@ -94,12 +119,13 @@
             dx = dx2d.view(n, ho, wo, cin).permute(0, 3, 1, 2)
             dw = e.tn2_wgrad(gy2d, x2d) if _wgrad2_enabled() \
                 else e.gemm_tn(gy2d, x2d, 0)
-        return dx, dw.reshape(cout, cin, 1, 1), None
+        return dx, dw.reshape(cout, cin, 1, 1), None, None
 
 
 def conv1x1_mfma(x: torch.Tensor, weight: torch.Tensor,
                  stride: int = 1) -> torch.Tensor:
-    y, stats = _Conv1x1.apply(x, weight, stride)
+    cell = getattr(x, "_amdtrain_tap_cell", None) if stride == 2 else None
+    y, stats = _Conv1x1.apply(x, weight, stride, cell)
     if stats.numel():
         y._amdtrain_bn_stats = stats
     return y
diff --git a/amdtrain/ops/csrc/batchnorm.hip b/amdtrain/ops/csrc/batchnorm.hip
--- a/amdtrain/ops/csrc/batchnorm.hip
+++ b/amdtrain/ops/csrc/batchnorm.hip
@@ -1,3 +1,6 @@
+#include <cstdlib>
+#include <cstring>
+
 #include "common.h"
 
 namespace {
@@ -10,8 +13,94 @@
   float* out = nullptr;
 };
 
+constexpr int GSRC_NONE = 0, GSRC_POOL = 1, GSRC_COMPACT = 2;
+
+template <typename T>
+struct BNGradSrc {
+  const T* gy = nullptr;
+  const T* gy2 = nullptr;
+  const unsigned char* idx = nullptr;
+  int H = 0, W = 0, Hs = 0, Ws = 0;
+};
+
+struct RowPos {
+  int n, h, w;
+};
+
+__device__ __forceinline__ RowPos row_decode(long r, int H, int W) {
+  RowPos p;
+  p.w = (int)(r % W);
+  r /= W;
+  p.h = (int)(r % H);
+  p.n = (int)(r / H);
+  return p;
+}
+
+__device__ __forceinline__ void row_advance(RowPos& p, const RowPos& d, int H,
+                                            int W) {
+  p.w += d.w;
+  int c = p.w >= W;
+  if (c) p.w -= W;
+  p.h += d.h + c;
+  c = p.h >= H;
+  if (c) p.h -= H;
+  p.n += d.n + c;
+}
+
+template <typename T, int VEC>
+__device__ __forceinline__ Pack<T, VEC> pool_grad_gather(
+    const BNGradSrc<T>& s, const RowPos& p, int C, int c0) {
+  float acc[VEC];
+#pragma unroll
+  for (int k = 0; k < VEC; ++k) acc[k] = 0.f;
+  const int nh = ((p.h & 1) && (p.h + 1) / 2 < s.Hs) ? 2 : 1;
+  const int nw = ((p.w & 1) && (p.w + 1) / 2 < s.Ws) ? 2 : 1;
+#pragma unroll
+  for (int a = 0; a < 2; ++a) {
+    if (a >= nh) continue;
+    const int ho = p.h / 2 + a;
+    const int kh = p.h - (ho * 2 - 1);
+#pragma unroll
+    for (int b = 0; b < 2; ++b) {
+      if (b >= nw) continue;
+      const int wo = p.w / 2 + b;
+      const int kw = p.w - (wo * 2 - 1);
+      const unsigned char code = (unsigned char)(kh * 3 + kw);
+      const long obase = (((long)p.n * s.Hs + ho) * s.Ws + wo) * C + c0;
+      Pack<unsigned char, VEC> iv =
+          *(const Pack<unsigned char, VEC>*)(s.idx + obase);
+      Pack<T, VEC> gv = *(const Pack<T, VEC>*)(s.gy + obase);
+      if (s.gy2 != nullptr) {
+        Pack<T, VEC> g2 = *(const Pack<T, VEC>*)(s.gy2 + obase);
+#pragma unroll
+        for (int k = 0; k < VEC; ++k)
+          gv.v[k] = from_f32<T>(to_f32(gv.v[k]) + to_f32(g2.v[k]));
+      }
+#pragma unroll
+      for (int k = 0; k < VEC; ++k)
+        if (iv.v[k] == code) acc[k] += to_f32(gv.v[k]);
+    }
+  }
+  Pack<T, VEC> out;
+#pragma unroll
+  for (int k = 0; k < VEC; ++k) out.v[k] = from_f32<T>(acc[k]);
+  return out;
+}
+
+template <typename T, int VEC>
+__device__ __forceinline__ Pack<T, VEC> compact_grad_gather(
+    const BNGradSrc<T>& s, const RowPos& p, int C, int c0) {
+  if (((p.h | p.w) & 1) == 0)
+    return *(const Pack<T, VEC>*)(
+        s.gy + (((long)p.n * s.Hs + p.h / 2) * s.Ws + p.w / 2) * C + c0);
+  Pack<T, VEC> z;
+#pragma unroll
+  for (int k = 0; k < VEC; ++k) z.v[k] = from_f32<T>(0.f);
+  return z;
+}
+
 template <typename T, int VEC, bool BWD, int MASK, bool WG, bool GO2,
-          bool DUAL = false>
+          bool DUAL = false, int GSRC = GSRC_NONE>
 __global__ void __launch_bounds__(AMD_TPB)
 bn_reduce_kernel(const T* __restrict__ x, const T* __restrict__ go,
                  const T* __restrict__ goB, const T* __restrict__ y,
@@ -20,8 +109,10 @@
                  const float* __restrict__ scale,
                  const float* __restrict__ shift, T* __restrict__ ghat_out,
                  float* __restrict__ out, long R, int C,
-                 BNDualSide<T> ds = {}) {
+                 BNDualSide<T> ds = {}, BNGradSrc<T> gs = {}) {
   static_assert(!DUAL || (BWD && WG), "DUAL rides the ghat-writing bwd pass");
+  static_assert(GSRC == GSRC_NONE || BWD, "gather operands are gradients");
+  static_assert(GSRC != GSRC_COMPACT || GO2, "the compact operand is go2");
   const int t = threadIdx.x;
   const int gpr = C / VEC;
   const long rows_per_block = (R + gridDim.x - 1) / gridDim.x;
@@ -54,15 +145,31 @@
         }
       }
     }
+    RowPos pos{0, 0, 0};
+    if (GSRC != GSRC_NONE && r0 + phase < r1)
+      pos = row_decode(r0 + phase, gs.H, gs.W);
     for (long r = r0 + phase; r < r1; r += rstep) {
       const long base = r * C + c0;
       Pack<T, VEC> xv = *(const Pack<T, VEC>*)(x + base);
       Pack<T, VEC> gv, gv2, yv, gh, dv;
       unsigned int mbits = 0;
       if (BWD) {
-        gv = *(const Pack<T, VEC>*)(go + base);
+        if (GSRC == GSRC_POOL) gv = pool_grad_gather<T, VEC>(gs, pos, C, c0);
+        else gv = *(const Pack<T, VEC>*)(go + base);
         if (DUAL) dv = *(const Pack<T, VEC>*)(ds.x + base);
-        if (GO2) gv2 = *(const Pack<T, VEC>*)(goB + base);
+        if (GSRC == GSRC_COMPACT)
+          gv2 = compact_grad_gather<T, VEC>(gs, pos, C, c0);
+        else if (GO2) gv2 = *(const Pack<T, VEC>*)(goB + base);
+        if (GSRC != GSRC_NONE) {
+          pos.w += rstep;
+          while (pos.w >= gs.W) {
+            pos.w -= gs.W;
+            if (++pos.h == gs.H) {
+              pos.h = 0;
+              ++pos.n;
+            }
+          }
+        }
         if (MASK == 1) yv = *(const Pack<T, VEC>*)(y + base);
         if (MASK == 3)
           mbits = ((const unsigned char*)y)[base / VEC];
@@ -259,7 +366,7 @@
 }
 
 template <typename T, int VEC, bool RELU, bool HAS_ADD, bool POW2,
-          bool DUAL = false>
+          bool DUAL = false, bool REGC = DUAL>
 __global__ void __launch_bounds__(AMD_TPB)
 bn_apply_kernel(const T* __restrict__ x, const T* __restrict__ z,
                 T* __restrict__ y, unsigned char* __restrict__ mask,
@@ -268,19 +375,23 @@
                 const float* __restrict__ scale_d = nullptr,
                 const float* __restrict__ shift_d = nullptr) {
   static_assert(!DUAL || (HAS_ADD && POW2), "DUAL normalizes the addend");
+  static_assert(!DUAL || REGC, "DUAL keeps its coefficients in registers");
+  static_assert(!REGC || POW2, "REGC needs a pow2 channel-group count");
   extern __shared__ float sm[];
   const int gpr = C / VEC;
   const long stride = (long)gridDim.x * blockDim.x;
   float rs[VEC], rb[VEC], rsd[VEC], rbd[VEC];
-  if (DUAL) {
+  if (REGC) {
     const int cf =
         (int)(((long)blockIdx.x * blockDim.x + threadIdx.x) & (gpr - 1)) * VEC;
 #pragma unroll
     for (int k = 0; k < VEC; ++k) {
       rs[k] = scale[cf + k];
       rb[k] = shift[cf + k];
-      rsd[k] = scale_d[cf + k];
-      rbd[k] = shift_d[cf + k];
+      if (DUAL) {
+        rsd[k] = scale_d[cf + k];
+        rbd[k] = shift_d[cf + k];
+      }
     }
   } else {
     for (int c = threadIdx.x; c < C; c += blockDim.x) {
@@ -306,7 +417,7 @@
     unsigned int mb = 0, mb2 = 0;
 #pragma unroll
     for (int k = 0; k < VEC; ++k) {
-      float v = DUAL ? rs[k] * to_f32(xv.v[k]) + rb[k]
+      float v = REGC ? rs[k] * to_f32(xv.v[k]) + rb[k]
                      : sm[c0 + k] * to_f32(xv.v[k]) + sm[C + c0 + k];
       if (HAS_ADD) {
         float ze = to_f32(zv.v[k]);
@@ -318,7 +429,7 @@
         v = fmaxf(v, 0.f);
       }
       yv.v[k] = from_f32<T>(v);
-      float v2 = DUAL ? rs[k] * to_f32(xv2.v[k]) + rb[k]
+      float v2 = REGC ? rs[k] * to_f32(xv2.v[k]) + rb[k]
                       : sm[c02 + k] * to_f32(xv2.v[k]) + sm[C + c02 + k];
       if (HAS_ADD) {
         float ze2 = to_f32(zv2.v[k]);
@@ -381,8 +492,16 @@
   const float* Dc = nullptr;
 };
 
+template <int MASK>
+__device__ __forceinline__ float bn_bwd_gx(float a, float b, float d,
+                                           float ge, float xe) {
+#pragma clang fp contract(off)
+  if (MASK == 2) return __builtin_fmaf(b, xe, a * ge) + d;
+  return __builtin_fmaf(a, ge, b * xe) + d;
+}
+
 template <typename T, int VEC, int MASK, bool WRITE_GHAT, bool POW2,
-          bool DUAL = false>
+          bool DUAL = false, bool REGC = false, bool POOLGO = false>
 __global__ void __launch_bounds__(AMD_TPB)
 bn_bwd_apply_kernel(const T* __restrict__ x, const T* __restrict__ go,
                     T* __restrict__ gx,
@@ -390,9 +509,11 @@
                     const float* __restrict__ Bc, const float* __restrict__ Dc,
                     const float* __restrict__ scale,
                     const float* __restrict__ shift, long total_vec, int C,
-                    BNDualBwdSide<T> ds = {}) {
+                    BNDualBwdSide<T> ds = {}, BNGradSrc<T> gs = {}) {
   static_assert(!DUAL || (MASK == 0 && POW2 && !WRITE_GHAT),
                 "DUAL consumes the materialized ghat");
+  static_assert(!REGC || (POW2 && !DUAL), "REGC is the single-BN form");
+  static_assert(!POOLGO || REGC, "POOLGO rides the register path");
   const int gpr = C / VEC;
   const long stride = (long)gridDim.x * blockDim.x;
   if (DUAL) {
@@ -436,6 +557,69 @@
       if (has2) {
         *(Pack<T, VEC>*)(gx + i2 * VEC) = out2;
         *(Pack<T, VEC>*)(ds.gx + i2 * VEC) = dout2;
+      }
+    }
+    return;
+  }
+  if (REGC) {
+    const long i0 = (long)blockIdx.x * blockDim.x + threadIdx.x;
+    const int c0 = (int)(i0 & (gpr - 1)) * VEC;
+    float ra[VEC], rb[VEC], rd[VEC], rsc[VEC], rsh[VEC];
+#pragma unroll
+    for (int k = 0; k < VEC; ++k) {
+      ra[k] = A[c0 + k];
+      rb[k] = Bc[c0 + k];
+      rd[k] = Dc[c0 + k];
+      if (MASK == 2) {
+        rsc[k] = scale[c0 + k];
+        rsh[k] = shift[c0 + k];
+      }
+    }
+    RowPos p1{0, 0, 0}, p2{0, 0, 0}, dstep{0, 0, 0};
+    if (POOLGO) {
+      const int lg = __builtin_ctz(gpr);
+      const long rstride = stride >> lg;
+      if (i0 < total_vec) p1 = row_decode(i0 >> lg, gs.H, gs.W);
+      p2 = p1;
+      row_advance(p2, row_decode(rstride, gs.H, gs.W), gs.H, gs.W);
+      dstep = row_decode(2 * rstride, gs.H, gs.W);
+    }
+    for (long i = i0; i < total_vec; i += 2 * stride) {
+      const bool has2 = i + stride < total_vec;
+      const long i2 = has2 ? i + stride : i;
+      Pack<T, VEC> xv = *(const Pack<T, VEC>*)(x + i * VEC);
+      Pack<T, VEC> xv2 = *(const Pack<T, VEC>*)(x + i2 * VEC);
+      Pack<T, VEC> gv, gv2;
+      if (POOLGO) {
+        gv = pool_grad_gather<T, VEC>(gs, p1, C, c0);
+        gv2 = pool_grad_gather<T, VEC>(gs, has2 ? p2 : p1, C, c0);
+        row_advance(p1, dstep, gs.H, gs.W);
+        row_advance(p2, dstep, gs.H, gs.W);
+      } else {
+        gv = *(const Pack<T, VEC>*)(go + i * VEC);
+        gv2 = *(const Pack<T, VEC>*)(go + i2 * VEC);
+      }
+      Pack<T, VEC> out, gh, out2, gh2;
+#pragma unroll
+      for (int k = 0; k < VEC; ++k) {
+        float xe = to_f32(xv.v[k]);
+        float ge = to_f32(gv.v[k]);
+        if (MASK == 2 && rsc[k] * xe + rsh[k] <= 0.f) ge = 0.f;
+        float v = bn_bwd_gx<MASK>(ra[k], rb[k], rd[k], ge, xe);
+        out.v[k] = from_f32<T>(v);
+        if (WRITE_GHAT) gh.v[k] = from_f32<T>(ge);
+        float xe2 = to_f32(xv2.v[k]);
+        float ge2 = to_f32(gv2.v[k]);
+        if (MASK == 2 && rsc[k] * xe2 + rsh[k] <= 0.f) ge2 = 0.f;
+        float v2 = bn_bwd_gx<MASK>(ra[k], rb[k], rd[k], ge2, xe2);
+        out2.v[k] = from_f32<T>(v2);
+        if (WRITE_GHAT) gh2.v[k] = from_f32<T>(ge2);
+      }
+      *(Pack<T, VEC>*)(gx + i * VEC) = out;
+      if (WRITE_GHAT) *(Pack<T, VEC>*)(ghat_out + i * VEC) = gh;
+      if (has2) {
+        *(Pack<T, VEC>*)(gx + i2 * VEC) = out2;
+        if (WRITE_GHAT) *(Pack<T, VEC>*)(ghat_out + i2 * VEC) = gh2;
       }
     }
     return;
@@ -510,6 +694,50 @@
         TORCH_CHECK(C / VEC <= 2 * AMD_TPB, "C too large: ", C);
         fn((devT*)nullptr, std::integral_constant<int, VEC>{});
       });
+}
+
+static bool bn_regcoef_enabled() {
+  const char* v = std::getenv("AMDTRAIN_BN_REGCOEF");
+  return v == nullptr || std::strcmp(v, "1") == 0;
+}
+
+static void bn_apply_launch(const at::Tensor& x,
+                            const std::optional<at::Tensor>& addend,
+                            at::Tensor& y, const at::Tensor& mask,
+                            const at::Tensor& scale, const at::Tensor& shift,
+                            bool relu) {
+  const long C = x.size(1);
+  const long R = x.numel() / C;
+  auto stream = at::cuda::getCurrentCUDAStream();
+  dispatch_vec(x, [&](auto* tp, auto vec) {
+    using devT = std::remove_pointer_t<decltype(tp)>;
+    constexpr int VEC = decltype(vec)::value;
+    long total_vec = R * C / VEC;
+    int agrid = amd_grid(total_vec);
+    const bool regc = bn_regcoef_enabled() && C / VEC <= AMD_TPB;
+    size_t smem = regc ? 0 : 2 * C * sizeof(float);
+    const devT* zp =
+        addend ? (const devT*)addend->const_data_ptr() : nullptr;
+#define APPLY(RELU_, ADD_, REGC_)                                           \
+  bn_apply_kernel<devT, VEC, RELU_, ADD_, true, false, REGC_>               \
+      <<<agrid, AMD_TPB, smem, stream>>>(                                   \
+          (const devT*)x.const_data_ptr(), zp, (devT*)y.data_ptr(),         \
+          mask.defined() ? mask.data_ptr<unsigned char>() : nullptr,        \
+          scale.data_ptr<float>(), shift.data_ptr<float>(), total_vec,      \
+          (int)C)
+#define APPLY_RC(RELU_, ADD_)                                               \
+  do {                                                                      \
+    if (regc) APPLY(RELU_, ADD_, true);                                     \
+    else APPLY(RELU_, ADD_, false);                                         \
+  } while (0)
+    if (relu && addend) APPLY_RC(true, true);
+    else if (relu) APPLY_RC(true, false);
+    else if (addend) APPLY_RC(false, true);
+    else APPLY_RC(false, false);
+#undef APPLY_RC
+#undef APPLY
+    CHECK_CUDA_OK();
+  });
 }
 
 static int bn_reduce_grid(long R, int C) {
@@ -601,6 +829,37 @@
   return k;
 }
 
+template <typename devT, int VEC>
+static void bn_bwd_apply_launch(const devT* x, const devT* go, devT* gx,
+                                const BNBwdCoeffs& k, const float* scp,
+                                const float* shp, long R, long C,
+                                const BNGradSrc<devT>* pool) {
+  auto stream = at::cuda::getCurrentCUDAStream();
+  const long total_vec = R * C / VEC;
+  const int agrid = amd_grid(total_vec);
+  const bool affine = scp != nullptr;
+  const bool fits = C / VEC <= AMD_TPB;
+#define BAPPLY(MASK_, REGC_, POOL_, SMEM_, GS_)                             \
+  bn_bwd_apply_kernel<devT, VEC, MASK_, false, true, false, REGC_, POOL_>   \
+      <<<agrid, AMD_TPB, SMEM_, stream>>>(                                  \
+          x, go, gx, nullptr, k.A.data_ptr<float>(),                        \
+          k.Bc.data_ptr<float>(), k.Dc.data_ptr<float>(), scp, shp,         \
+          total_vec, (int)C, BNDualBwdSide<devT>{}, GS_)
+  if (pool != nullptr) {
+    TORCH_CHECK(affine && fits, "pool-gather bwd apply: unsupported form");
+    BAPPLY(2, true, true, 0, *pool);
+  } else if (bn_regcoef_enabled() && fits) {
+    if (affine) BAPPLY(2, true, false, 0, BNGradSrc<devT>{});
+    else BAPPLY(0, true, false, 0, BNGradSrc<devT>{});
+  } else {
+    const size_t smem = (affine ? 5 : 3) * C * sizeof(float);
+    if (affine) BAPPLY(2, false, false, smem, BNGradSrc<devT>{});
+    else BAPPLY(0, false, false, smem, BNGradSrc<devT>{});
+  }
+#undef BAPPLY
+  CHECK_CUDA_OK();
+}
+
 static void check_dual(const at::Tensor& x3, const at::Tensor& x_d) {
   check_nhwc(x3);
   check_nhwc(x_d);
@@ -634,34 +893,11 @@
   at::Tensor mask;
   if (relu && addend)
     mask = at::empty({R * C / 4}, x.options().dtype(at::kByte));
-  auto stream = at::cuda::getCurrentCUDAStream();
   auto st = bn_train_stats(x, std::nullopt, weight, bias, running_mean,
                            running_var, momentum, eps);
   auto &mean = st.mean, &invstd = st.invstd, &scale = st.scale,
        &shift = st.shift;
-
-  dispatch_vec(x, [&](auto* tp, auto vec) {
-    using devT = std::remove_pointer_t<decltype(tp)>;
-    constexpr int VEC = decltype(vec)::value;
-    long total_vec = R * C / VEC;
-    int agrid = amd_grid(total_vec);
-    size_t smem = 2 * C * sizeof(float);
-    const devT* zp =
-        addend ? (const devT*)addend->const_data_ptr() : nullptr;
-#define APPLY(RELU_, ADD_)                                                  \
-  bn_apply_kernel<devT, VEC, RELU_, ADD_, true>                             \
-      <<<agrid, AMD_TPB, smem, stream>>>(                                   \
-          (const devT*)x.const_data_ptr(), zp, (devT*)y.data_ptr(),         \
-          mask.defined() ? mask.data_ptr<unsigned char>() : nullptr,        \
-          scale.data_ptr<float>(), shift.data_ptr<float>(),     \
-          total_vec, (int)C)
-    if (relu && addend) APPLY(true, true);
-    else if (relu) APPLY(true, false);
-    else if (addend) APPLY(false, true);
-    else APPLY(false, false);
-#undef APPLY
-    CHECK_CUDA_OK();
-  });
+  bn_apply_launch(x, addend, y, mask, scale, shift, relu);
   if (!mask.defined()) mask = at::empty({0}, x.options().dtype(at::kByte));
   return {y, mean, invstd, scale, shift, mask};
 }
@@ -677,33 +913,11 @@
   at::Tensor mask;
   if (relu && addend)
     mask = at::empty({R * C / 4}, x.options().dtype(at::kByte));
-  auto stream = at::cuda::getCurrentCUDAStream();
   auto st = bn_train_stats(x, parts, weight, bias, running_mean, running_var,
                            momentum, eps);
   auto &mean = st.mean, &invstd = st.invstd, &scale = st.scale,
        &shift = st.shift;
-  dispatch_vec(x, [&](auto* tp, auto vec) {
-    using devT = std::remove_pointer_t<decltype(tp)>;
-    constexpr int VEC = decltype(vec)::value;
-    long total_vec = R * C / VEC;
-    int agrid = amd_grid(total_vec);
-    size_t smem = 2 * C * sizeof(float);
-    const devT* zp =
-        addend ? (const devT*)addend->const_data_ptr() : nullptr;
-#define APPLY2(RELU_, ADD_)                                                 \
-  bn_apply_kernel<devT, VEC, RELU_, ADD_, true>                             \
-      <<<agrid, AMD_TPB, smem, stream>>>(                                   \
-          (const devT*)x.const_data_ptr(), zp, (devT*)y.data_ptr(),         \
-          mask.defined() ? mask.data_ptr<unsigned char>() : nullptr,        \
-          scale.data_ptr<float>(), shift.data_ptr<float>(),                 \
-          total_vec, (int)C)
-    if (relu && addend) APPLY2(true, true);
-    else if (relu) APPLY2(true, false);
-    else if (addend) APPLY2(false, true);
-    else APPLY2(false, false);
-#undef APPLY2
-    CHECK_CUDA_OK();
-  });
+  bn_apply_launch(x, addend, y, mask, scale, shift, relu);
   if (!mask.defined()) mask = at::empty({0}, x.options().dtype(at::kByte));
   return {y, mean, invstd, scale, shift, mask};
 }
@@ -818,28 +1032,7 @@
       running_mean.data_ptr<float>(), running_var.data_ptr<float>(),
       scale.data_ptr<float>(), shift.data_ptr<float>(), (int)C, (float)eps);
   CHECK_CUDA_OK();
-  dispatch_vec(x, [&](auto* tp, auto vec) {
-    using devT = std::remove_pointer_t<decltype(tp)>;
-    constexpr int VEC = decltype(vec)::value;
-    long total_vec = R * C / VEC;
-    int agrid = amd_grid(total_vec);
-    size_t smem = 2 * C * sizeof(float);
-    const devT* zp =
-        addend ? (const devT*)addend->const_data_ptr() : nullptr;
-#define APPLY(RELU_, ADD_)                                                  \
-  bn_apply_kernel<devT, VEC, RELU_, ADD_, true>                             \
-      <<<agrid, AMD_TPB, smem, stream>>>(                                   \
-          (const devT*)x.const_data_ptr(), zp, (devT*)y.data_ptr(),         \
-          mask.defined() ? mask.data_ptr<unsigned char>() : nullptr,        \
-          scale.data_ptr<float>(), shift.data_ptr<float>(),     \
-          total_vec, (int)C)
-    if (relu && addend) APPLY(true, true);
-    else if (relu) APPLY(true, false);
-    else if (addend) APPLY(false, true);
-    else APPLY(false, false);
-#undef APPLY
-    CHECK_CUDA_OK();
-  });
+  bn_apply_launch(x, addend, y, mask, scale, shift, relu);
   return y;
 }
 
@@ -851,7 +1044,8 @@
                                        std::optional<at::Tensor> scale,
                                        std::optional<at::Tensor> shift,
                                        std::optional<at::Tensor> grad_out2,
-                                       std::optional<at::Tensor> relu_mask) {
+                                       std::optional<at::Tensor> relu_mask,
+                                       bool grad_out2_compact) {
   check_nhwc(x);
   check_nhwc(grad_out);
   const long C = x.size(1);
@@ -866,6 +1060,23 @@
   at::Tensor ghat;
   if (mask_y || grad_out2) ghat = at::empty_like(grad_out);
   auto stream = at::cuda::getCurrentCUDAStream();
+  const long H = x.size(2), W = x.size(3);
+  const long Hs = (H + 1) / 2, Ws = (W + 1) / 2;
+  if (grad_out2_compact) {
+    TORCH_CHECK(grad_out2.has_value() && grad_out2->is_cuda() &&
+                    grad_out2->dim() == 2 && grad_out2->is_contiguous() &&
+                    grad_out2->scalar_type() == x.scalar_type() &&
+                    grad_out2->size(0) == x.size(0) * Hs * Ws &&
+                    grad_out2->size(1) == C,
+                "batch_norm_bwd: compact grad_out2 must be a contiguous "
+                "[N*ceil(H/2)*ceil(W/2), C] tensor of x's dtype");
+    TORCH_CHECK(C * (long)x.element_size() / 16 <= AMD_TPB,
+                "batch_norm_bwd: C too wide for a compact grad_out2: ", C);
+  } else if (grad_out2) {
+    check_nhwc(*grad_out2);
+    TORCH_CHECK(grad_out2->sizes() == x.sizes(),
+                "batch_norm_bwd: grad_out2 shape mismatch");
+  }
 
   dispatch_vec(x, [&](auto* tp, auto vec) {
     using devT = std::remove_pointer_t<decltype(tp)>;
@@ -874,31 +1085,42 @@
     const float* shp = affine_mask ? shift->data_ptr<float>() : nullptr;
     const devT* go2p = grad_out2
         ? (const devT*)grad_out2->const_data_ptr() : nullptr;
-#define REDUCE(MASK_, WG_, GO2_)                                            \
-  bn_reduce_kernel<devT, VEC, true, MASK_, WG_, GO2_>                       \
+    BNGradSrc<devT> gs;
+    if (grad_out2_compact) {
+      gs.gy = go2p;
+      gs.H = (int)H, gs.W = (int)W, gs.Hs = (int)Hs, gs.Ws = (int)Ws;
+    }
+#define REDUCE_G(MASK_, WG_, GO2_, GSRC_)                                   \
+  bn_reduce_kernel<devT, VEC, true, MASK_, WG_, GO2_, false, GSRC_>         \
       <<<rgrid, AMD_TPB, 0, stream>>>(                                      \
           (const devT*)x.const_data_ptr(),                                  \
           (const devT*)grad_out.const_data_ptr(), go2p,                     \
           yp, mean.data_ptr<float>(),                                       \
           invstd.data_ptr<float>(), scp, shp,                               \
           WG_ ? (devT*)ghat.data_ptr() : nullptr,                           \
-          sums.data_ptr<float>(), R, (int)C)
-#define REDUCE3(GO2_)                                                       \
-  bn_reduce_kernel<devT, VEC, true, 3, true, GO2_>                          \
+          sums.data_ptr<float>(), R, (int)C, BNDualSide<devT>{}, gs)
+#define REDUCE(MASK_, WG_, GO2_) REDUCE_G(MASK_, WG_, GO2_, GSRC_NONE)
+#define REDUCE3_G(GO2_, GSRC_)                                              \
+  bn_reduce_kernel<devT, VEC, true, 3, true, GO2_, false, GSRC_>            \
       <<<rgrid, AMD_TPB, 0, stream>>>(                                      \
           (const devT*)x.const_data_ptr(),                                  \
           (const devT*)grad_out.const_data_ptr(), go2p,                     \
           (const devT*)mkp, mean.data_ptr<float>(),                         \
           invstd.data_ptr<float>(), scp, shp,                               \
           (devT*)ghat.data_ptr(),                                           \
-          sums.data_ptr<float>(), R, (int)C)
+          sums.data_ptr<float>(), R, (int)C, BNDualSide<devT>{}, gs)
+#define REDUCE3(GO2_) REDUCE3_G(GO2_, GSRC_NONE)
     const unsigned char* mkp = (relu_mask && relu_mask->numel())
         ? relu_mask->data_ptr<unsigned char>() : nullptr;
     TORCH_CHECK(y.has_value() || !mask_y || mkp,
                 "batch_norm_bwd: y is required to mask a relu+addend BN "
                 "that saved no relu_mask");
     const devT* yp = y ? (const devT*)y->const_data_ptr() : nullptr;
-    if (mask_y && mkp && go2p) REDUCE3(true);
+    if (grad_out2_compact) {
+      if (mask_y && mkp) REDUCE3_G(true, GSRC_COMPACT);
+      else if (mask_y) REDUCE_G(1, true, true, GSRC_COMPACT);
+      else REDUCE_G(0, true, true, GSRC_COMPACT);
+    } else if (mask_y && mkp && go2p) REDUCE3(true);
     else if (mask_y && mkp) REDUCE3(false);
     else if (mask_y && go2p) REDUCE(1, true, true);
     else if (mask_y) REDUCE(1, true, false);
@@ -907,25 +1129,75 @@
     else REDUCE(0, false, false);
 #undef REDUCE
 #undef REDUCE3
+#undef REDUCE_G
+#undef REDUCE3_G
     CHECK_CUDA_OK();
     k = bn_bwd_coeffs(sums, weight, mean, invstd, R, C);
-    long total_vec = R * C / VEC;
-    int agrid = amd_grid(total_vec);
-    size_t smem = (affine_mask ? 5 : 3) * C * sizeof(float);
     const devT* go_in = ghat.defined()
                             ? (const devT*)ghat.const_data_ptr()
                             : (const devT*)grad_out.const_data_ptr();
-#define BAPPLY(MASK_)                                                       \
-  bn_bwd_apply_kernel<devT, VEC, MASK_, false, true>                        \
-      <<<agrid, AMD_TPB, smem, stream>>>(                                   \
-          (const devT*)x.const_data_ptr(), go_in, (devT*)gx.data_ptr(),     \
-          nullptr, k.A.data_ptr<float>(), k.Bc.data_ptr<float>(),           \
-          k.Dc.data_ptr<float>(), scp, shp, total_vec, (int)C)
-    if (affine_mask) BAPPLY(2);
-    else BAPPLY(0);
-#undef BAPPLY
-    CHECK_CUDA_OK();
+    bn_bwd_apply_launch<devT, VEC>((const devT*)x.const_data_ptr(), go_in,
+                                   (devT*)gx.data_ptr(), k, scp, shp, R, C,
+                                   nullptr);
   });
   if (!ghat.defined()) ghat = grad_out;
   return {gx, k.gw, k.gb, ghat};
 }
+
+std::vector<at::Tensor> batch_norm_bwd_pool(
+    at::Tensor x, at::Tensor grad_pool, std::optional<at::Tensor> grad_pool2,
+    at::Tensor idx, at::Tensor weight, at::Tensor mean, at::Tensor invstd,
+    at::Tensor scale, at::Tensor shift) {
+  check_nhwc(x);
+  check_nhwc(grad_pool);
+  const long N = x.size(0), C = x.size(1), H = x.size(2), W = x.size(3);
+  const long Ho = (H - 1) / 2 + 1, Wo = (W - 1) / 2 + 1;
+  const long R = N * H * W;
+  const std::vector<int64_t> pool_shape{N, C, Ho, Wo};
+  TORCH_CHECK(grad_pool.sizes() == pool_shape &&
+                  grad_pool.scalar_type() == x.scalar_type(),
+              "batch_norm_bwd_pool: grad_pool must be [N,C,Ho,Wo] of x's "
+              "dtype");
+  TORCH_CHECK(idx.is_cuda() && idx.scalar_type() == at::kByte &&
+                  idx.sizes() == pool_shape &&
+                  idx.is_contiguous(at::MemoryFormat::ChannelsLast),
+              "batch_norm_bwd_pool: idx must be NHWC u8 [N,C,Ho,Wo]");
+  if (grad_pool2) {
+    check_nhwc(*grad_pool2);
+    TORCH_CHECK(grad_pool2->sizes() == pool_shape &&
+                    grad_pool2->scalar_type() == x.scalar_type(),
+                "batch_norm_bwd_pool: grad_pool2 shape/dtype mismatch");
+  }
+  TORCH_CHECK(C * (long)x.element_size() / 16 <= AMD_TPB,
+              "batch_norm_bwd_pool: C too wide for the register path: ", C);
+  TORCH_CHECK(R < (1L << 31), "batch_norm_bwd_pool: too many rows");
+  auto opts = x.options().dtype(at::kFloat);
+  const int rgrid = bn_reduce_grid(R, C);
+  auto sums = at::empty({rgrid, 2 * C}, opts);
+  BNBwdCoeffs k;
+  auto gx = at::empty_like(x);
+  auto stream = at::cuda::getCurrentCUDAStream();
+  dispatch_vec(x, [&](auto* tp, auto vec) {
+    using devT = std::remove_pointer_t<decltype(tp)>;
+    constexpr int VEC = decltype(vec)::value;
+    const float* scp = scale.data_ptr<float>();
+    const float* shp = shift.data_ptr<float>();
+    BNGradSrc<devT> gs;
+    gs.gy = (const devT*)grad_pool.const_data_ptr();
+    gs.gy2 = grad_pool2 ? (const devT*)grad_pool2->const_data_ptr() : nullptr;
+    gs.idx = idx.data_ptr<unsigned char>();
+    gs.H = (int)H, gs.W = (int)W, gs.Hs = (int)Ho, gs.Ws = (int)Wo;
+    bn_reduce_kernel<devT, VEC, true, 2, false, false, false, GSRC_POOL>
+        <<<rgrid, AMD_TPB, 0, stream>>>(
+            (const devT*)x.const_data_ptr(), nullptr, nullptr, nullptr,
+            mean.data_ptr<float>(), invstd.data_ptr<float>(), scp, shp,
+            nullptr, sums.data_ptr<float>(), R, (int)C, BNDualSide<devT>{},
+            gs);
+    CHECK_CUDA_OK();
+    k = bn_bwd_coeffs(sums, weight, mean, invstd, R, C);
+    bn_bwd_apply_launch<devT, VEC>((const devT*)x.const_data_ptr(), nullptr,
+                                   (devT*)gx.data_ptr(), k, scp, shp, R, C,
+                                   &gs);
+  });
+  return {gx, k.gw, k.gb};
+}
diff --git a/amdtrain/ops/csrc/ext.cpp b/amdtrain/ops/csrc/ext.cpp
--- a/amdtrain/ops/csrc/ext.cpp
+++ b/amdtrain/ops/csrc/ext.cpp
@@ -59,7 +59,12 @@
                                        std::optional<at::Tensor> scale,
                                        std::optional<at::Tensor> shift,
                                        std::optional<at::Tensor> grad_out2,
-                                       std::optional<at::Tensor> relu_mask);
+                                       std::optional<at::Tensor> relu_mask,
+                                       bool grad_out2_compact);
+std::vector<at::Tensor> batch_norm_bwd_pool(
+    at::Tensor x, at::Tensor grad_pool, std::optional<at::Tensor> grad_pool2,
+    at::Tensor idx, at::Tensor weight, at::Tensor mean, at::Tensor invstd,
+    at::Tensor scale, at::Tensor shift);
 
 at::Tensor gemm_bt(at::Tensor A, at::Tensor B, bool f32_out,
                    std::optional<at::Tensor> addend,
@@ -142,7 +147,12 @@
         py::arg("relu"), py::arg("need_ghat"),
         py::arg("scale") = std::nullopt, py::arg("shift") = std::nullopt,
         py::arg("grad_out2") = std::nullopt,
-        py::arg("relu_mask") = std::nullopt);
+        py::arg("relu_mask") = std::nullopt,
+        py::arg("grad_out2_compact") = false);
+  m.def("batch_norm_bwd_pool", &batch_norm_bwd_pool, py::arg("x"),
+        py::arg("grad_pool"), py::arg("grad_pool2"), py::arg("idx"),
+        py::arg("weight"), py::arg("mean"), py::arg("invstd"),
+        py::arg("scale"), py::arg("shift"));
   m.def("gemm_bt", &gemm_bt, py::arg("A"), py::arg("B"),
         py::arg("f32_out") = false, py::arg("addend") = std::nullopt,
         py::arg("bias") = std::nullopt);
diff --git a/amdtrain/ops/fused.py b/amdtrain/ops/fused.py
--- a/amdtrain/ops/fused.py
+++ b/amdtrain/ops/fused.py
@@ -8,7 +8,7 @@
 import torch.nn.functional as F
 
 from ._ext import require_ext, use_ext_for
-from .conv import GradCell
+from .conv import GradCell, _dsgrad_compact_enabled
 
 __all__ = ["batch_norm", "bn_add_relu", "bn_add_relu_downsample",
            "bn_relu_max_pool", "max_pool_3x3_s2", "global_avg_pool"]
@@ -40,15 +40,19 @@
     def backward(ctx, grad_out):
         x, y, weight, mean, invstd, scale, shift, mask = ctx.saved_tensors
         e = require_ext()
-        go2 = None
+        go2, compact = None, False
         cell = getattr(ctx, "res_cell", None)
         if cell is not None and cell.g is not None:
-            go2 = cell.g.contiguous(memory_format=torch.channels_last)
+            if cell.meta is not None:
+                go2, compact = cell.g.contiguous(), True
+            else:
+                go2 = cell.g.contiguous(memory_format=torch.channels_last)
             cell.g = None
+            cell.meta = None
         grad_x, grad_w, grad_b, ghat = e.batch_norm_bwd(
             x, grad_out.contiguous(memory_format=torch.channels_last),
             y, weight, mean, invstd, ctx.relu, ctx.has_addend,
-            scale, shift, go2, mask)
+            scale, shift, go2, mask, compact)
         grad_addend = ghat if ctx.has_addend else None
         return (grad_x, grad_w, grad_b, None, None, None, None, None,
                 grad_addend, None, None)
@@ -78,6 +82,9 @@
         ac = None if addend is None else addend.contiguous(memory_format=torch.channels_last)
         if bn.training:
             cell = GradCell() if (relu and ac is not None) else None
+            if cell is not None:
+                cell.compact_ok = (_dsgrad_compact_enabled()
+                                   and _vec_ok(xc, 256))
             out = _BNFunction.apply(xc, bn.weight, bn.bias, bn.running_mean,
                                     bn.running_var, bn.momentum, bn.eps,
                                     relu, ac, parts, cell)
@@ -136,6 +143,10 @@
 
 def _stemfuse_enabled() -> bool:
     return os.environ.get("AMDTRAIN_STEMFUSE", "1") == "1"
+
+
+def _poolbwd_fuse_enabled() -> bool:
+    return os.environ.get("AMDTRAIN_POOLBWD_FUSE", "1") == "1"
 
 
 def _vec_ok(x: torch.Tensor, max_groups: int) -> bool:
@@ -197,26 +208,37 @@
 
     @staticmethod
     def forward(ctx, x, weight, bias, running_mean, running_var, momentum,
-                eps, parts):
+                eps, parts, res_cell=None):
         e = require_ext()
         mean, invstd, scale, shift = e.batch_norm_train_stats(
             x, parts, weight, bias, running_mean, running_var,
             float(momentum), float(eps))
         y, idx = e.max_pool_3x3_s2_fwd(x, scale, shift)
         ctx.save_for_backward(x, idx, weight, mean, invstd, scale, shift)
+        ctx.res_cell = res_cell
         return y
 
     @staticmethod
     def backward(ctx, grad_out):
         x, idx, weight, mean, invstd, scale, shift = ctx.saved_tensors
         e = require_ext()
-        gp = e.max_pool_3x3_s2_bwd(
-            grad_out.contiguous(memory_format=torch.channels_last), idx,
-            int(x.size(2)), int(x.size(3)))
-        grad_x, grad_w, grad_b, _ = e.batch_norm_bwd(
-            x, gp, None, weight, mean, invstd, True, False, scale, shift,
-            None, None)
-        return grad_x, grad_w, grad_b, None, None, None, None, None
+        go = grad_out.contiguous(memory_format=torch.channels_last)
+        cell = getattr(ctx, "res_cell", None)
+        if cell is not None:
+            go2 = None
+            if cell.g is not None:
+                go2 = cell.g.to(go.dtype).contiguous(
+                    memory_format=torch.channels_last)
+                cell.g = None
+            grad_x, grad_w, grad_b = e.batch_norm_bwd_pool(
+                x, go, go2, idx, weight, mean, invstd, scale, shift)
+        else:
+            gp = e.max_pool_3x3_s2_bwd(go, idx, int(x.size(2)),
+                                       int(x.size(3)))
+            grad_x, grad_w, grad_b, _ = e.batch_norm_bwd(
+                x, gp, None, weight, mean, invstd, True, False, scale,
+                shift, None, None)
+        return grad_x, grad_w, grad_b, None, None, None, None, None, None
 
 
 def bn_relu_max_pool(x: torch.Tensor, bn) -> torch.Tensor:
@@ -225,10 +247,15 @@
         if bn.track_running_stats and bn.num_batches_tracked is not None:
             bn.num_batches_tracked.add_(1)
         parts = getattr(x, "_amdtrain_bn_stats", None)
-        return _BNReLUMaxPool.apply(
+        cell = GradCell() if (_poolbwd_fuse_enabled()
+                              and _vec_ok(x, 256)) else None
+        out = _BNReLUMaxPool.apply(
             x.contiguous(memory_format=torch.channels_last), bn.weight,
             bn.bias, bn.running_mean, bn.running_var, bn.momentum, bn.eps,
-            parts)
+            parts, cell)
+        if cell is not None:
+            out._amdtrain_next_cell = cell
+        return out
     return max_pool_3x3_s2(batch_norm(x, bn, relu=True))
 
 
```

After: 10460 images/sec, median of 6. +3.1%, better.
